# yjxiong/action-detection

Hardware: NVIDIA H100
Metric: proposals/sec (9-seg BNInception SSN fwd+bwd) (higher is better)
Workload: dtype f32 via split f16 operands (hi+lo, 3 wgmma MMAs per product) / f32 accumulate; f32 storage

## Files before the change

### action-detection_b200/csrc/engine.cu

```cuda
#include <cstdio>
#include <cstdlib>
#include <algorithm>
#include <cstring>
#include <map>
#include <string>
#include <vector>

#include <cuda_profiler_api.h>

#include "../../include/ssnb.h"
#include "common.cuh"
#include "umma_conv.cuh"

namespace ssnb {

std::atomic<long long> g_launches{0};
static thread_local std::string t_error;
void set_thread_error(const std::string& s) { t_error = s; }
const std::string& thread_error() { return t_error; }

thread_local bool t_timing = false;
thread_local LaunchTag t_tag;
struct TimingMark { const char* what; LaunchTag tag; std::string op; cudaEvent_t ev; };
static thread_local std::vector<TimingMark> t_marks;
static thread_local std::vector<cudaEvent_t> t_event_pool;
static thread_local std::string t_report;
static cudaEvent_t timing_event() {
  if (!t_event_pool.empty()) { cudaEvent_t e = t_event_pool.back(); t_event_pool.pop_back(); return e; }
  cudaEvent_t e = nullptr;
  cudaEventCreate(&e);
  return e;
}
void timing_mark(const char* what, cudaStream_t s) {
  TimingMark m{what, t_tag, t_tag.op ? t_tag.op : "", timing_event()};
  m.tag.op = nullptr;
  if (m.ev && cudaEventRecord(m.ev, s) == cudaSuccess) t_marks.push_back(m);
  else cudaGetLastError();
  t_tag.flop = 0.0; t_tag.op = nullptr; t_tag.tiles = 0; t_tag.block_n = 0;
}

static bool timing_close() {
  t_timing = false;
  if (t_marks.empty()) return false;
  if (cudaEventSynchronize(t_marks.back().ev) != cudaSuccess) { cudaGetLastError(); return false; }
  return true;
}

struct BlockSpec { const char* name; int c1, c3r, c3, cdr, cd1, cd2; int pool_max; int cproj; int stride; };
static const BlockSpec kBlocks[10] = {
    {"3a", 64, 64, 64, 64, 96, 96, 0, 32, 1},      {"3b", 64, 64, 96, 64, 96, 96, 0, 64, 1},
    {"3c", 0, 128, 160, 64, 96, 96, 1, 0, 2},      {"4a", 224, 64, 96, 96, 128, 128, 0, 128, 1},
    {"4b", 192, 96, 128, 96, 128, 128, 0, 128, 1}, {"4c", 160, 128, 160, 128, 160, 160, 0, 128, 1},
    {"4d", 96, 128, 192, 160, 192, 192, 0, 128, 1}, {"4e", 0, 128, 192, 192, 256, 256, 1, 0, 2},
    {"5a", 352, 192, 320, 160, 224, 224, 0, 128, 1}, {"5b", 352, 192, 320, 192, 224, 224, 1, 128, 1}};

struct ConvSpec { std::string id; int cin, cout, k, stride, pad; };

static std::vector<ConvSpec> conv_table(int in_ch) {
  std::vector<ConvSpec> v;
  v.push_back({"conv1_7x7_s2", in_ch, 64, 7, 2, 3});
  v.push_back({"conv2_3x3_reduce", 64, 64, 1, 1, 0});
  v.push_back({"conv2_3x3", 64, 192, 3, 1, 1});
  int cx = 192;
  for (const BlockSpec& b : kBlocks) {
    std::string p = std::string("inception_") + b.name + "_";
    if (b.c1) v.push_back({p + "1x1", cx, b.c1, 1, 1, 0});
    v.push_back({p + "3x3_reduce", cx, b.c3r, 1, 1, 0});
    v.push_back({p + "3x3", b.c3r, b.c3, 3, b.stride, 1});
    v.push_back({p + "double_3x3_reduce", cx, b.cdr, 1, 1, 0});
    v.push_back({p + "double_3x3_1", b.cdr, b.cd1, 3, 1, 1});
    v.push_back({p + "double_3x3_2", b.cd1, b.cd2, 3, b.stride, 1});
    if (b.cproj) v.push_back({p + "pool_proj", cx, b.cproj, 1, 1, 0});
    cx = b.c1 + b.c3 + b.cd2 + (b.cproj ? b.cproj : cx);
  }
  return v;
}

struct Buffer { std::string name; int H, W, C; size_t off = 0, goff = 0; size_t hoff = 0, ghoff = 0, plane = 0; };
struct Value { std::string name; int buf, coff, C; };
enum OpKind { OP_CONV = 0, OP_MAXPOOL = 1, OP_AVGPOOL = 2, OP_GPOOL = 3, OP_BN1 = 4 };
struct Op {
  OpKind kind; std::string id; int in_val, out_val;
  int conv = -1, k = 0, stride = 1, pad = 0;
  size_t argmax_off = 0;
  int grad_accumulate = 0;
  int wsplits = 1, wrows = 0;
  int tsplits = 1;
  size_t partial_off = 0, bias_partial_off = 0;
  UmmaConvPlan umma;
  UmmaConvPlan umma_dgrad;
  UmmaWgradPlan umma_wgrad;
  int pool_consumer = -1;
  bool folded_into_conv = false;
  bool dgrad_masks = false;
  bool bias_in_wgrad = false;
  bool dy_premasked = false;
  bool raw = false;
  int fuse_role = 0;
  int fuse_block = -1;
};
struct PackedConv { size_t wf, wd, bias, scale; size_t wf16 = 0, wd16 = 0, wplane = 0, wmax = 0; };
struct FusedBlock {
  int op1 = -1, op_r3 = -1, op_rd = -1;
  int c1 = 0, c3r = 0, cdr = 0, cx = 0;
  size_t w_fwd = 0, bias = 0, w_dg = 0;
  size_t w_fwd_plane = 0, w_dg_plane = 0, wmax = 0;
  UmmaConvPlan fwd, dgrad;
  bool enabled = false;
};

}

using namespace ssnb;

struct ssnb_engine {
  ssnb_config cfg;
  int F = 0;
  size_t esz = 4;
  size_t up_plane = 0, s2d_plane = 0, s2d_w_plane = 0;
  int* tc_flag = nullptr;
  size_t tc_flag_off = 0, wmax_off = 0;
  bool bn1_train = false;
  const float *bn1_gamma = nullptr, *bn1_beta = nullptr; float *bn1_rmean = nullptr, *bn1_rvar = nullptr, *bn1_dgamma = nullptr, *bn1_dbeta = nullptr;
  float bn1_momentum = 0.1f, bn1_eps = 1e-5f;
  size_t bn_stat_off = 0, bn_partial_off = 0;
  std::vector<ConvSpec> convs;
  std::vector<Buffer> bufs;
  std::vector<Value> vals;
  std::map<std::string, int> val_by_name;
  std::vector<Op> ops;
  std::vector<PackedConv> packed;
  std::vector<FusedBlock> fused;
  size_t ws_bytes = 0, partial_off = 0, partial_bytes = 0, bpartial_off = 0;
  size_t s2d_off = 0, s2d_w_off = 0, up_off = 0;
  bool fold_pools = true;
  bool s2d_ready = false;
  int Cs = 0;
  char* ws = nullptr;
  bool weights_ready = false;
  std::vector<float*> dw, db;
  std::vector<int> pending_finalize;
  int grad_accumulate = 0;
  std::string error;
  long long launches0 = 0;
  UmmaContext umma_ctx;

  int fail(int code, const std::string& msg) { error = msg; return code; }
  bool fast() const { return cfg.precision == SSNB_FAST_FP16; }
  bool exact_tc() const { return cfg.precision == SSNB_EXACT_TC; }
  bool tensor_cores() const { return cfg.precision != SSNB_EXACT_FP32; }
  int nplanes() const { return exact_tc() ? 2 : 1; }
  View view(int val, bool grad) const {
    const Value& v = vals[val];
    const Buffer& b = bufs[v.buf];
    View w;
    w.base = ws + (grad ? b.goff : b.off);
    w.H = b.H; w.W = b.W; w.C = v.C; w.pitch = b.C; w.coff = v.coff;
    return w;
  }
  View planes(int val, bool grad) const {
    const Value& v = vals[val];
    const Buffer& b = bufs[v.buf];
    View w;
    w.base = ws + (grad ? b.ghoff : b.hoff);
    w.H = b.H; w.W = b.W; w.C = v.C; w.pitch = b.C; w.coff = v.coff; w.lo_off = (long long)b.plane;
    return w;
  }
  View operand(int val, bool grad) const { return exact_tc() ? planes(val, grad) : view(val, grad); }
  const __half* w_fwd(const PackedConv& p) const { return (const __half*)(ws + (exact_tc() ? p.wd16 : p.wd)); }
  const __half* w_dgrad(const PackedConv& p) const { return (const __half*)(ws + (exact_tc() ? p.wf16 : p.wf)); }
  const UmmaTcOpts* tc_opts(UmmaTcOpts& t, size_t w_lo_off, void* out32, float alpha, size_t wmax) const {
    if (!exact_tc()) return nullptr;
    t.w_lo_off = (long long)w_lo_off; t.out32 = (float*)out32; t.alpha = alpha; t.alpha_dev = (const float*)(ws + wmax) + 1;
    return &t;
  }
};

namespace ssnb {

static size_t align_up(size_t v, size_t a) { return (v + a - 1) / a * a; }
static bool profiled_op(const char* env, const std::string& id) {
  const char* e = getenv(env);
  if (!e || !*e) return false;
  const std::string list = std::string(",") + e + ",";
  return list.find("," + id + ",") != std::string::npos;
}
static bool env_on(const char* name) {
  const char* v = getenv(name);
  return v && v[0] == '1';
}
static int device_sms() {
  int dev = 0, sms = 0;
  if (cudaGetDevice(&dev) != cudaSuccess || cudaDeviceGetAttribute(&sms, cudaDevAttrMultiProcessorCount, dev) != cudaSuccess || sms <= 0) {
    cudaGetLastError();
    return 132;
  }
  return sms;
}

static int pool_out(int h, int k, int s, int p) {
  int o = (h + 2 * p - k + s - 1) / s + 1;
  if ((o - 1) * s >= h + p) --o;
  return o;
}

static int add_buffer(ssnb_engine* e, const std::string& name, int H, int W, int C) {
  e->bufs.push_back({name, H, W, C});
  return (int)e->bufs.size() - 1;
}
static int add_value(ssnb_engine* e, const std::string& name, int buf, int coff, int C) {
  e->vals.push_back({name, buf, coff, C});
  e->val_by_name[name] = (int)e->vals.size() - 1;
  return (int)e->vals.size() - 1;
}

static void build_graph(ssnb_engine* e) {
  const int cin = e->cfg.in_channels;
  e->convs = conv_table(cin);
  int ci = 0;
  auto conv_op = [&](int in_val, int out_val) {
    const ConvSpec& c = e->convs[ci];
    Op o; o.kind = OP_CONV; o.id = c.id; o.in_val = in_val; o.out_val = out_val; o.conv = ci;
    o.k = c.k; o.stride = c.stride; o.pad = c.pad;
    e->ops.push_back(o);
    ++ci;
  };
  auto pool_op = [&](OpKind kind, const std::string& id, int in_val, int out_val, int k, int s, int p) {
    Op o; o.kind = kind; o.id = id; o.in_val = in_val; o.out_val = out_val; o.k = k; o.stride = s; o.pad = p;
    e->ops.push_back(o);
  };
  auto whole = [&](const std::string& name, int H, int W, int C) {
    return add_value(e, name, add_buffer(e, name, H, W, C), 0, C);
  };
  int x = whole("data", 224, 224, cin);
  int v;
  if (e->bn1_train) {
    const int raw = whole("conv1_7x7_s2_raw", 112, 112, 64); conv_op(x, raw); e->ops.back().raw = true;
    v = whole("conv1_7x7_s2_bn", 112, 112, 64);
    pool_op(OP_BN1, "conv1_7x7_s2_bn", raw, v, 0, 1, 0); x = v;
  } else {
    v = whole("conv1_7x7_s2_bn", 112, 112, 64); conv_op(x, v); x = v;
  }
  v = whole("pool1_3x3_s2", 56, 56, 64); pool_op(OP_MAXPOOL, "pool1_3x3_s2", x, v, 3, 2, 0); x = v;
  v = whole("conv2_3x3_reduce_bn", 56, 56, 64); conv_op(x, v); x = v;
  v = whole("conv2_3x3_bn", 56, 56, 192); conv_op(x, v); x = v;
  v = whole("pool2_3x3_s2", 28, 28, 192); pool_op(OP_MAXPOOL, "pool2_3x3_s2", x, v, 3, 2, 0); x = v;
  int H = 28, cx = 192;
  for (const BlockSpec& b : kBlocks) {
    const std::string p = std::string("inception_") + b.name + "_";
    const int OHW = (b.stride == 2) ? pool_out(H, 3, 2, 0) : H;
    const int ctot = b.c1 + b.c3 + b.cd2 + (b.cproj ? b.cproj : cx);
    const int cat = add_buffer(e, p + "output", OHW, OHW, ctot);
    const int red = add_buffer(e, p + "reduce", H, H, b.c3r + b.cdr);
    int off = 0;
    if (b.c1) { v = add_value(e, p + "1x1_bn", cat, off, b.c1); conv_op(x, v); off += b.c1; }
    int r3 = add_value(e, p + "3x3_reduce_bn", red, 0, b.c3r); conv_op(x, r3);
    v = add_value(e, p + "3x3_bn", cat, off, b.c3); conv_op(r3, v); off += b.c3;
    int rd = add_value(e, p + "double_3x3_reduce_bn", red, b.c3r, b.cdr); conv_op(x, rd);
    int d1 = whole(p + "double_3x3_1_bn", H, H, b.cd1); conv_op(rd, d1);
    v = add_value(e, p + "double_3x3_2_bn", cat, off, b.cd2); conv_op(d1, v); off += b.cd2;
    if (b.stride == 2) {
      v = add_value(e, p + "pool", cat, off, cx);
      pool_op(OP_MAXPOOL, p + "pool", x, v, 3, 2, 0);
    } else {
      int pl = whole(p + "pool", H, H, cx);
      pool_op(b.pool_max ? OP_MAXPOOL : OP_AVGPOOL, p + "pool", x, pl, 3, 1, 1);
      v = add_value(e, p + "pool_proj_bn", cat, off, b.cproj); conv_op(pl, v);
    }
    x = add_value(e, p + "output", cat, 0, ctot);
    H = OHW; cx = ctot;
  }
  Op g; g.kind = OP_GPOOL; g.id = "global_pool"; g.in_val = x; g.out_val = -1; g.k = 7;
  e->ops.push_back(g);
}

static void plan(ssnb_engine* e) {
  const size_t F = (size_t)e->F;
  size_t off = 0;
  for (Buffer& b : e->bufs) { b.off = off; off = align_up(off + F * b.H * b.W * b.C * e->esz, 1024); }
  if (e->cfg.training)
    for (Buffer& b : e->bufs) { b.goff = off; off = align_up(off + F * b.H * b.W * b.C * e->esz, 1024); }
  if (e->exact_tc()) {
    for (Buffer& b : e->bufs) {
      if (b.C % 8) continue;
      b.plane = align_up(F * b.H * b.W * b.C * 2, 1024);
      b.hoff = off; off += 2 * b.plane;
      if (e->cfg.training) { b.ghoff = off; off += 2 * b.plane; }
    }
  }
  e->tc_flag_off = off; off = align_up(off + 256, 1024);
  if (e->bn1_train) { e->bn_stat_off = off; off = align_up(off + 4 * 64 * 4, 1024); e->bn_partial_off = off; off = align_up(off + (size_t)1200 * 2 * 64 * 4, 1024); }
  for (Op& o : e->ops)
    if (o.kind == OP_MAXPOOL) {
      const Buffer& ob = e->bufs[e->vals[o.out_val].buf];
      o.argmax_off = off;
      off = align_up(off + F * ob.H * ob.W * e->vals[o.out_val].C, 1024);
    }
  e->packed.resize(e->convs.size());
  for (size_t i = 0; i < e->convs.size(); ++i) {
    const ConvSpec& c = e->convs[i];
    const size_t n = (size_t)c.cout * c.cin * c.k * c.k;
    e->packed[i].wf = off; off = align_up(off + n * e->esz, 1024);
    e->packed[i].wd = off; off = align_up(off + n * e->esz, 1024);
    e->packed[i].bias = off; off = align_up(off + c.cout * 4, 256);
    e->packed[i].scale = off; off = align_up(off + c.cout * 4, 256);
    if (e->exact_tc()) {
      e->packed[i].wplane = align_up(n * 2, 1024);
      e->packed[i].wf16 = off; off += 2 * e->packed[i].wplane;
      e->packed[i].wd16 = off; off += 2 * e->packed[i].wplane;
    }
  }
  if (e->exact_tc()) {
    e->wmax_off = off;
    for (size_t i = 0; i < e->convs.size(); ++i) e->packed[i].wmax = off + i * 8;
    off = align_up(off + (e->convs.size() + 16) * 8, 1024);
  }
  size_t pmax = 0;
  if (e->cfg.training) {
    std::vector<char> written(e->vals.size(), 0);
    for (int i = (int)e->ops.size() - 1; i >= 0; --i) {
      Op& o = e->ops[i];
      o.grad_accumulate = written[o.in_val];
      written[o.in_val] = 1;
      if (o.kind == OP_CONV) {
        const ConvSpec& c = e->convs[o.conv];
        const Buffer& ob = e->bufs[e->vals[o.out_val].buf];
        const long long M = (long long)F * ob.H * ob.W;
        const int taps = c.k * c.k;
        const bool flat = c.cin < 16;
        const long long tiles = (long long)((c.cout + 63) / 64) * (flat ? (taps * c.cin + 63) / 64 : ((c.cin + 63) / 64) * taps);
        long long splits = (592 + tiles - 1) / tiles;
        if (splits > 128) splits = 128;
        while (splits > 1 && M / splits < 256) --splits;
        long long rows = (M + splits - 1) / splits;
        rows = (rows + 15) / 16 * 16;
        splits = (M + rows - 1) / rows;
        o.wsplits = (int)splits; o.wrows = (int)rows;
        {
          const int chunks = (c.cin + 63) / 64, n_tiles = (chunks + 3) / 4, block_n = ((chunks + n_tiles - 1) / n_tiles) * 64;
          const int tpc = std::max(1, 4 / (block_n / 64));
          const int ctas = ((c.cout + 127) / 128) * n_tiles * ((taps + tpc - 1) / tpc);
          o.tsplits = std::max(o.wsplits, std::min(128, std::max(1, device_sms() / ctas)));
        }
        if (e->tensor_cores()) splits = std::max<long long>(splits, o.tsplits);
        const size_t need = (size_t)splits * taps * c.cout * c.cin * 4;
        if (need > pmax) pmax = need;
      }
    }
  }
  if (e->tensor_cores()) {
    for (int i = 0; i < (int)e->ops.size(); ++i) {
      const Op& o = e->ops[i];
      if (o.kind != OP_CONV || o.k != 1) continue;
      const std::string& id = o.id;
      const std::string suf = "_3x3_reduce";
      if (id.size() < suf.size() || id.compare(id.size() - suf.size(), suf.size(), suf) != 0 || id.find("double") != std::string::npos) continue;
      const std::string pre = id.substr(0, id.size() - suf.size() + 1);
      FusedBlock fb; fb.op_r3 = i;
      for (int j = 0; j < (int)e->ops.size(); ++j) {
        if (e->ops[j].id == pre + "1x1") fb.op1 = j;
        if (e->ops[j].id == pre + "double_3x3_reduce") fb.op_rd = j;
      }
      if (fb.op_rd < 0) continue;
      fb.cx = e->convs[o.conv].cin; fb.c3r = e->convs[o.conv].cout; fb.cdr = e->convs[e->ops[fb.op_rd].conv].cout;
      fb.c1 = fb.op1 >= 0 ? e->convs[e->ops[fb.op1].conv].cout : 0;
      const int n = fb.c1 + fb.c3r + fb.cdr, kf = (fb.c1 + 63) / 64 * 64 + fb.c3r + fb.cdr;
      fb.w_fwd_plane = align_up((size_t)n * fb.cx * 2, 1024); fb.w_dg_plane = align_up((size_t)fb.cx * kf * 2, 1024);
      if (e->exact_tc()) fb.w_fwd_plane = fb.w_dg_plane = std::max(fb.w_fwd_plane, fb.w_dg_plane);
      fb.w_fwd = off; off += e->nplanes() * fb.w_fwd_plane;
      fb.bias = off; off = align_up(off + (size_t)n * 4, 256);
      fb.w_dg = off; off += e->nplanes() * fb.w_dg_plane;
      if (e->exact_tc()) {
        if (e->fused.size() >= 16) continue;
        fb.wmax = e->wmax_off + (e->convs.size() + e->fused.size()) * 8;
        for (int j : {fb.op1, fb.op_r3, fb.op_rd}) if (j >= 0) e->packed[e->ops[j].conv].wmax = fb.wmax;
      }
      e->fused.push_back(fb);
    }
  }
  if (e->tensor_cores()) {
    for (int i = 0; i < (int)e->ops.size(); ++i) {
      Op& po = e->ops[i];
      if (po.kind != OP_MAXPOOL || po.k != 3 || po.stride != 2 || po.pad != 0) continue;
      int producer = -1, consumers = 0;
      for (int j = 0; j < (int)e->ops.size(); ++j) {
        if (e->ops[j].out_val == po.in_val && e->ops[j].kind == OP_CONV) producer = j;
        if (e->ops[j].in_val == po.in_val) ++consumers;
      }
      if (producer >= 0 && consumers == 1 && e->vals[po.in_val].C % (e->fast() ? 8 : 4) == 0) { e->ops[producer].pool_consumer = i; po.folded_into_conv = true; }
    }
    auto operand_region = [&](size_t bytes, size_t& plane) {
      const size_t at = off;
      if (e->exact_tc()) { plane = align_up(bytes, 1024); off += 2 * plane; }
      else off = align_up(off + bytes, 1024);
      return at;
    };
    e->Cs = (4 * e->cfg.in_channels + 7) / 8 * 8;
    e->s2d_off = operand_region(F * 112 * 112 * 4 * e->Cs * 2, e->s2d_plane);
    e->s2d_w_off = operand_region((size_t)16 * 64 * e->Cs * 2, e->s2d_w_plane);
    if (e->cfg.training) {
      size_t up = 0;
      for (const Op& o : e->ops)
        if (o.kind == OP_CONV && o.stride == 2 && o.conv != 0) {
          const Buffer& ib = e->bufs[e->vals[o.in_val].buf];
          up = std::max(up, F * ib.H * ib.W * (size_t)e->convs[o.conv].cout * 2);
        }
      e->up_off = operand_region(up, e->up_plane);
      pmax = std::max(pmax, (size_t)128 * 16 * 64 * e->Cs * 4);
    }
  }
  e->partial_off = off; e->partial_bytes = pmax; off = align_up(off + pmax, 1024);
  if (e->cfg.training)
    for (Op& o : e->ops)
      if (o.kind == OP_CONV) {
        const ConvSpec& c = e->convs[o.conv];
        const int nsplit = e->tensor_cores() ? std::max(o.wsplits, o.tsplits) : o.wsplits;
        size_t need = (size_t)nsplit * c.k * c.k * c.cout * c.cin * 4;
        if (o.conv == 0 && e->tensor_cores()) need = std::max(need, (size_t)128 * 16 * 64 * e->Cs * 4);
        o.partial_off = off; off = align_up(off + need, 1024);
        o.bias_partial_off = off; off = align_up(off + (size_t)std::max(nsplit, 128) * c.cout * 4, 256);
      }
  e->bpartial_off = off; off = align_up(off + (size_t)1024 * 512 * 4, 1024);
  e->ws_bytes = off;
}

#define DISPATCH(e, call_f, call_h) ((e)->fast() ? (call_h) : (call_f))

static double conv_flops(const ssnb_engine* e, const Op& o) {
  const ConvSpec& c = e->convs[o.conv];
  const Buffer& ob = e->bufs[e->vals[o.out_val].buf];
  return 2.0 * e->F * ob.H * ob.W * (double)c.cout * c.cin * c.k * c.k;
}
static inline void tag_next(int phase, double flop, const char* op = nullptr) { t_tag.phase = phase; t_tag.flop = flop; t_tag.op = op; }
static thread_local std::string t_fused_name;
static const char* fused_name(const ssnb_engine* e, const FusedBlock& fb) {
  if (!t_timing) return nullptr;
  t_fused_name.clear();
  for (int j : {fb.op1, fb.op_r3, fb.op_rd})
    if (j >= 0) t_fused_name += (t_fused_name.empty() ? "" : "+") + e->ops[j].id;
  return t_fused_name.c_str();
}

static int tc_split_value(ssnb_engine* e, int val, bool grad, float scale, cudaStream_t s) {
  if (!e->exact_tc() || !e->bufs[e->vals[val].buf].plane) return 0;
  return launch_split_view(e->view(val, grad), e->F, scale, e->planes(val, grad), grad ? e->tc_flag : nullptr, s);
}

static int run_fwd_impl(ssnb_engine* e, const Op& o, const float* input_nchw, float* feat, cudaStream_t s);
static int run_fwd(ssnb_engine* e, const Op& o, const float* input_nchw, float* feat, cudaStream_t s) {
  tag_next(0, 0.0);
  if (o.kind == OP_CONV && o.umma.enabled) {
    if (o.conv == 0 && !e->s2d_ready) {
      const View in = e->view(o.in_val, false);
      __half* s2d = (__half*)(e->ws + e->s2d_off);
      if (int rc = e->exact_tc() ? launch_nhwc_to_s2d_split(in, e->F, s2d, (long long)e->s2d_plane, e->Cs, s) : launch_nhwc_to_s2d(in, e->F, s2d, e->Cs, s))
        return rc;
    }
    tag_next(0, conv_flops(e, o), o.id.c_str());
    return umma_conv_launch(e->umma_ctx, o.umma, s);
  }
  if (o.kind == OP_BN1) {
    if (!e->bn1_gamma || !e->bn1_beta) { set_thread_error("bn1_train engine: call ssnb_set_bn1 first"); return SSNB_ESTATE; }
    return launch_bn_train_fwd(e->view(o.in_val, false), e->view(o.out_val, false), e->exact_tc() ? e->planes(o.out_val, false) : View(), e->F, e->bn1_gamma,
                               e->bn1_beta, e->bn1_eps, e->bn1_momentum, e->bn1_rmean, e->bn1_rvar, (float*)(e->ws + e->bn_stat_off),
                               (float*)(e->ws + e->bn_partial_off), 1200, s);
  }
  if (e->exact_tc() && (o.kind == OP_MAXPOOL || o.kind == OP_AVGPOOL) && e->bufs[e->vals[o.out_val].buf].plane) {
    const View in = e->view(o.in_val, false), out = e->view(o.out_val, false), pl = e->planes(o.out_val, false);
    if (o.kind == OP_MAXPOOL) return launch_maxpool_fwd_f4(in, out, pl, e->F, o.k, o.stride, o.pad, (uint8_t*)(e->ws + o.argmax_off), s);
    return launch_avgpool3_f4(in, out, pl, e->F, 0, s);
  }
  if (int rc = run_fwd_impl(e, o, input_nchw, feat, s)) return rc;
  return o.out_val >= 0 ? tc_split_value(e, o.out_val, false, 1.0f, s) : 0;
}

static int run_fwd_impl(ssnb_engine* e, const Op& o, const float* input_nchw, float* feat, cudaStream_t s) {
  const int F = e->F;
  if (o.kind == OP_CONV) {
    const ConvSpec& c = e->convs[o.conv];
    const View in = e->view(o.in_val, false), out = e->view(o.out_val, false);
    ConvArgs a;
    a.src = in.base; a.SH = in.H; a.SW = in.W; a.Csrc = in.C; a.src_pitch = in.pitch; a.src_coff = in.coff;
    a.dst = out.base; a.DH = out.H; a.DW = out.W; a.Cdst = out.C; a.dst_pitch = out.pitch; a.dst_coff = out.coff;
    a.wgt = e->ws + e->packed[o.conv].wf; a.bias = (const float*)(e->ws + e->packed[o.conv].bias);
    a.F = F; a.k = c.k; a.stride = c.stride; a.pad = c.pad; a.relu = o.raw ? 0 : 1; a.accumulate = 0; a.dgrad = 0;
    tag_next(0, conv_flops(e, o), o.id.c_str());
    return DISPATCH(e, launch_conv<float>(a, s), launch_conv<__half>(a, s));
  }
  if (o.kind == OP_MAXPOOL) {
    const View in = e->view(o.in_val, false), out = e->view(o.out_val, false);
    uint8_t* am = (uint8_t*)(e->ws + o.argmax_off);
    if (e->fast() && in.C % 8 == 0) return launch_maxpool_fwd_h8(in, out, F, o.k, o.stride, o.pad, am, s);
    return DISPATCH(e, launch_maxpool_fwd<float>(in, out, F, o.k, o.stride, o.pad, am, s),
                    launch_maxpool_fwd<__half>(in, out, F, o.k, o.stride, o.pad, am, s));
  }
  if (o.kind == OP_AVGPOOL) {
    const View in = e->view(o.in_val, false), out = e->view(o.out_val, false);
    if (e->fast() && in.C % 8 == 0) return launch_avgpool3_h8(in, out, F, 0, s);
    return DISPATCH(e, launch_avgpool3_fwd<float>(in, out, F, 0, s), launch_avgpool3_fwd<__half>(in, out, F, 0, s));
  }
  if (o.kind == OP_GPOOL) {
    if (!feat) return e->fail(SSNB_EINVAL, "global_pool needs the feat output pointer");
    const View in = e->view(o.in_val, false);
    return DISPATCH(e, launch_gpool_fwd<float>(in, F, feat, s), launch_gpool_fwd<__half>(in, F, feat, s));
  }
  return SSNB_EINVAL;
}

static int simt_wgrad(ssnb_engine* e, const Op& o, cudaStream_t s) {
  const ConvSpec& c = e->convs[o.conv];
  const View x = e->view(o.in_val, false), dz = e->view(o.out_val, true);
  float* partial = (float*)(e->ws + o.partial_off);
  WgradArgs w;
  w.dz = dz.base; w.OH = dz.H; w.OW = dz.W; w.Cout = dz.C; w.dz_pitch = dz.pitch; w.dz_coff = dz.coff;
  w.x = x.base; w.IH = x.H; w.IW = x.W; w.Cin = x.C; w.x_pitch = x.pitch; w.x_coff = x.coff;
  w.partial = partial; w.F = e->F; w.k = c.k; w.stride = c.stride; w.pad = c.pad;
  w.rows_per_split = o.wrows; w.splits = o.wsplits;
  tag_next(2, conv_flops(e, o), o.id.c_str());
  if (int rc = DISPATCH(e, launch_wgrad<float>(w, s), launch_wgrad<__half>(w, s))) return rc;
  const float out_scale = e->fast() ? 1.0f / e->cfg.grad_scale : 1.0f;
  return launch_wgrad_finalize(partial, o.wsplits, c.k * c.k, c.cout, c.cin, (const float*)(e->ws + e->packed[o.conv].scale), out_scale,
                               e->dw[o.conv], e->grad_accumulate, s);
}
static int simt_dgrad(ssnb_engine* e, const Op& o, cudaStream_t s) {
  const ConvSpec& c = e->convs[o.conv];
  const View dz = e->view(o.out_val, true), dx = e->view(o.in_val, true);
  ConvArgs a;
  a.src = dz.base; a.SH = dz.H; a.SW = dz.W; a.Csrc = dz.C; a.src_pitch = dz.pitch; a.src_coff = dz.coff;
  a.dst = dx.base; a.DH = dx.H; a.DW = dx.W; a.Cdst = dx.C; a.dst_pitch = dx.pitch; a.dst_coff = dx.coff;
  a.wgt = e->ws + e->packed[o.conv].wd; a.bias = nullptr;
  a.F = e->F; a.k = c.k; a.stride = c.stride; a.pad = c.pad; a.relu = 0; a.accumulate = o.grad_accumulate; a.dgrad = 1;
  tag_next(1, conv_flops(e, o), o.id.c_str());
  return DISPATCH(e, launch_conv<float>(a, s), launch_conv<__half>(a, s));
}

static int run_bwd(ssnb_engine* e, const Op& o, const float* dfeat, cudaStream_t s, bool skip_dgrad = false, bool full = false) {
  const int F = e->F;
  const float gs = e->fast() ? e->cfg.grad_scale : 1.0f;
  int rc = 0;
  tag_next(3, 0.0);
  if (o.kind == OP_GPOOL) {
    if (!dfeat) return e->fail(SSNB_EINVAL, "global_pool backward needs dfeat");
    const View din = e->view(o.in_val, true);
    const void* ym = (full && e->fold_pools && o.dgrad_masks) ? e->view(o.in_val, false).base : nullptr;
    return DISPATCH(e, launch_gpool_bwd<float>(dfeat, gs, din, F, ym, s), launch_gpool_bwd<__half>(dfeat, gs, din, F, ym, s));
  }
  if (o.kind == OP_BN1) {
    return launch_bn_train_bwd(e->view(o.in_val, false), e->view(o.out_val, true), e->view(o.out_val, false), e->view(o.in_val, true),
                               e->exact_tc() ? e->planes(o.in_val, true) : View(), e->cfg.grad_scale, e->tc_flag, F, e->bn1_gamma, (float*)(e->ws + e->bn_stat_off),
                               (float*)(e->ws + e->bn_partial_off), 1200, e->bn1_dgamma, e->bn1_dbeta, e->grad_accumulate, s);
  }
  if (o.kind == OP_MAXPOOL) {
    if (full && e->tensor_cores() && e->fold_pools && o.folded_into_conv) return 0;
    const View din = e->view(o.in_val, true), dout = e->view(o.out_val, true);
    const uint8_t* am = (const uint8_t*)(e->ws + o.argmax_off);
    if (e->exact_tc() && din.C % 4 == 0) return launch_maxpool_bwd_f4(din, dout, F, o.k, o.stride, o.pad, am, o.grad_accumulate, s);
    if (e->fast() && din.C % 8 == 0) return launch_maxpool_bwd_h8(din, dout, F, o.k, o.stride, o.pad, am, o.grad_accumulate, s);
    return DISPATCH(e, launch_maxpool_bwd<float>(din, dout, F, o.k, o.stride, o.pad, am, o.grad_accumulate, s),
                    launch_maxpool_bwd<__half>(din, dout, F, o.k, o.stride, o.pad, am, o.grad_accumulate, s));
  }
  if (o.kind == OP_AVGPOOL) {
    const View din = e->view(o.in_val, true), dout = e->view(o.out_val, true);
    if (e->exact_tc() && din.C % 4 == 0) return launch_avgpool3_f4(dout, din, View(), F, o.grad_accumulate, s);
    if (e->fast() && din.C % 8 == 0) return launch_avgpool3_h8(dout, din, F, o.grad_accumulate, s);
    return DISPATCH(e, launch_avgpool3_fwd<float>(dout, din, F, o.grad_accumulate, s),
                    launch_avgpool3_fwd<__half>(dout, din, F, o.grad_accumulate, s));
  }
  const ConvSpec& c = e->convs[o.conv];
  const View x = e->view(o.in_val, false), y = e->view(o.out_val, false), dy = e->view(o.out_val, true);
  const float* scale = (const float*)(e->ws + e->packed[o.conv].scale);
  float* bpartial = (float*)(e->ws + e->bpartial_off);
  float* dbp = (e->db.size() && e->db[o.conv]) ? e->db[o.conv] : nullptr;
  const bool want_w = e->dw.size() && e->dw[o.conv];
  const bool want_x = e->vals[o.in_val].name != "data" && !skip_dgrad;
  if (!e->tensor_cores()) {
    if (!o.raw && (rc = launch_relu_mask<float>(dy, y, F, s))) return rc;
    if (dbp) {
      const long long M = (long long)F * y.H * y.W;
      int bs = (int)((M + 4095) / 4096); if (bs > 64) bs = 64; if (bs < 1) bs = 1;
      if ((rc = launch_bias_grad<float>(dy.base, (int)M, y.C, dy.pitch, dy.coff, scale, 1.0f, bpartial, bs, dbp, e->grad_accumulate, s))) return rc;
    }
    if (want_w && (rc = simt_wgrad(e, o, s))) return rc;
    return want_x ? simt_dgrad(e, o, s) : 0;
  }

  const float gst = e->cfg.grad_scale;
  const bool tc_w = want_w && o.umma_wgrad.enabled, tc_x = want_x && o.umma_dgrad.enabled;
  const bool pre = full && e->fold_pools && o.dy_premasked;
  const bool bias_w = pre && o.bias_in_wgrad && dbp && tc_w;
  const Op* pool = (full && e->fold_pools && o.pool_consumer >= 0) ? &e->ops[o.pool_consumer] : nullptr;
  const int max_ctas = (1024 * 512 - 64) / y.C;
  if (e->fast()) {
    if (pool) rc = launch_pool_mask_bias_h8(dy, y, e->view(pool->out_val, true), F, pool->k, pool->stride, pool->pad, (const uint8_t*)(e->ws + pool->argmax_off),
                                            scale, 1.0f / gst, bpartial, max_ctas, dbp, e->grad_accumulate, s);
    else if (!bias_w) rc = launch_mask_bias_h8(dy, pre ? View() : y, F, scale, 1.0f / gst, bpartial, max_ctas, dbp, e->grad_accumulate, s);
  } else {
    const bool need_f32 = (want_w && !tc_w) || (want_x && !tc_x);
    const View pl = (tc_w || tc_x) ? e->planes(o.out_val, true) : View();
    if (o.raw) {
      if (dbp) rc = launch_mask_bias_split_f4(dy, View(), View(), gst, 0, nullptr, F, scale, 1.0f, bpartial, max_ctas, dbp, e->grad_accumulate, s);
    } else if (pre) {
      if (!bias_w && dbp) rc = launch_mask_bias_split_f4(dy, y, View(), gst, 0, nullptr, F, scale, 1.0f, bpartial, max_ctas, dbp, e->grad_accumulate, s);
    } else if (pool) {
      rc = launch_pool_mask_bias_split_f4(dy, y, e->view(pool->out_val, true), pl, gst, need_f32 ? 1 : 0, e->tc_flag, F, (const uint8_t*)(e->ws + pool->argmax_off),
                                          scale, 1.0f, bpartial, max_ctas, dbp, e->grad_accumulate, s);
    } else {
      rc = launch_mask_bias_split_f4(dy, y, pl, gst, (need_f32 || !full) ? 1 : 0, e->tc_flag, F, scale, 1.0f, bpartial, max_ctas, dbp, e->grad_accumulate, s);
    }
  }
  if (rc) return rc;
  if (tc_x && c.stride == 2 && o.conv != 0) {
    View dz = e->operand(o.out_val, true);
    for (int p = 0; p < e->nplanes(); ++p, dz.base = (char*)dz.base + dz.lo_off)
      if ((rc = launch_upsample2_zero(dz, (__half*)(e->ws + e->up_off + p * e->up_plane), x.H, x.W, F, s))) return rc;
  }
  if (tc_w) {
    float* partial = (float*)(e->ws + o.partial_off);
    float* bp = bias_w ? (float*)(e->ws + o.bias_partial_off) : nullptr;
    tag_next(2, conv_flops(e, o), o.id.c_str());
    if ((rc = umma_wgrad_launch(e->umma_ctx, o.umma_wgrad, s, bp))) return rc;
    if (full && o.conv != 0) e->pending_finalize.push_back((int)(&o - e->ops.data()));
    else if (o.conv == 0) rc = launch_wgrad_finalize_s2d(partial, o.umma_wgrad.p.splits, c.cout, c.cin, e->Cs, scale, 1.0f / gst, e->dw[o.conv], e->grad_accumulate, s);
    else rc = launch_wgrad_finalize(partial, o.umma_wgrad.p.splits, c.k * c.k, c.cout, c.cin, scale, 1.0f / gst, e->dw[o.conv], e->grad_accumulate, s,
                                    nullptr, nullptr, e->tc_flag);
    if (rc) return rc;
  } else if (want_w && (rc = simt_wgrad(e, o, s))) return rc;
  if (tc_x) {
    tag_next(1, conv_flops(e, o), o.id.c_str());
    return umma_conv_launch(e->umma_ctx, o.umma_dgrad, s, full && e->fold_pools && o.dgrad_masks);
  }
  return want_x ? simt_dgrad(e, o, s) : 0;
}

int engine_tail_view(ssnb_handle h, View* v, int* F, int* fp16) {
  if (!h->ws || !h->weights_ready) return h->fail(SSNB_ESTATE, "workspace/weights not set");
  *v = h->view(h->ops.back().in_val, false);
  *F = h->F; *fp16 = h->fast() ? 1 : 0;
  return 0;
}

}

extern "C" {

const char* ssnb_version(void) { return "libssn_b200 0.3 (sm_90a)"; }

const char* ssnb_last_error(ssnb_handle h) { return h ? h->error.c_str() : ssnb::thread_error().c_str(); }

int ssnb_num_convs(void) { return 69; }

int ssnb_conv_info(int idx, int in_channels, char* name, int name_cap, int* cin, int* cout, int* k, int* stride, int* pad) {
  std::vector<ConvSpec> t = conv_table(in_channels);
  if (idx < 0 || idx >= (int)t.size()) { set_thread_error("ssnb_conv_info: index out of range"); return SSNB_EINVAL; }
  if (name && name_cap > 0) { snprintf(name, name_cap, "%s", t[idx].id.c_str()); }
  if (cin) *cin = t[idx].cin; if (cout) *cout = t[idx].cout; if (k) *k = t[idx].k;
  if (stride) *stride = t[idx].stride; if (pad) *pad = t[idx].pad;
  return SSNB_OK;
}

int ssnb_create(const ssnb_config* cfg, ssnb_handle* out) {
  if (!cfg || !out) { set_thread_error("ssnb_create: null argument"); return SSNB_EINVAL; }
  if (cfg->frames <= 0 || cfg->in_channels <= 0 || cfg->in_channels > 64) { set_thread_error("ssnb_create: bad frames/in_channels"); return SSNB_EINVAL; }
  if (cfg->precision != SSNB_EXACT_FP32 && cfg->precision != SSNB_FAST_FP16 && cfg->precision != SSNB_EXACT_TC) { set_thread_error("ssnb_create: unknown precision"); return SSNB_EINVAL; }
  ssnb_engine* e = new ssnb_engine();
  e->cfg = *cfg;
  if (!(e->cfg.grad_scale > 0.f)) e->cfg.grad_scale = 1.0f;
  e->F = cfg->frames;
  e->bn1_train = cfg->bn1_train != 0;
  if (e->bn1_train && e->fast()) { delete e; set_thread_error("ssnb_create: bn1_train (bn_mode='partial') needs EXACT_FP32 or EXACT_TC"); return SSNB_ENOSUPPORT; }
  e->esz = e->fast() ? 2 : 4;
  build_graph(e);
  if ((int)e->convs.size() != 69) { delete e; set_thread_error("internal: conv table size"); return SSNB_ESTATE; }
  umma_context_init(e->umma_ctx);
  plan(e);
  e->launches0 = g_launches.load();
  *out = e;
  return SSNB_OK;
}

int ssnb_destroy(ssnb_handle h) {
  if (!h) return SSNB_OK;
  umma_context_destroy(h->umma_ctx);
  delete h;
  return SSNB_OK;
}

size_t ssnb_workspace_bytes(ssnb_handle h) { return h ? h->ws_bytes : 0; }

int ssnb_set_workspace(ssnb_handle h, void* dev_ptr, size_t bytes) {
  if (!h) return SSNB_EINVAL;
  if (!dev_ptr || bytes < h->ws_bytes) return h->fail(SSNB_EINVAL, "workspace too small");
  if (((uintptr_t)dev_ptr) % 1024) return h->fail(SSNB_EINVAL, "workspace must be 1024-byte aligned");
  h->ws = (char*)dev_ptr;
  h->weights_ready = false;
  if (h->tensor_cores() && cudaMemset(h->ws + h->bpartial_off, 0, 256) != cudaSuccess) { cudaGetLastError();  }
  h->tc_flag = (int*)(h->ws + h->tc_flag_off);
  if (cudaMemset(h->tc_flag, 0, 256) != cudaSuccess) cudaGetLastError();
  const bool training = h->cfg.training != 0;
  const bool use_tc = h->tensor_cores() && !env_on("SSNB_DISABLE_UMMA");
  const bool use_wgrad = use_tc && training && !env_on("SSNB_DISABLE_UMMA_WGRAD");
  const bool fuse = !env_on("SSNB_DISABLE_FUSION");
  const float gs = h->cfg.grad_scale;
  for (Op& o : h->ops) {
    o.umma.enabled = o.umma_dgrad.enabled = o.umma_wgrad.enabled = false;
    o.fuse_role = 0; o.fuse_block = -1; o.dgrad_masks = o.dy_premasked = o.bias_in_wgrad = false;
  }
  for (FusedBlock& fb : h->fused) fb.enabled = false;
  h->fold_pools = fuse && (h->fast() || (use_tc && training));
  auto tc_gate = [&](UmmaConvPlan& p) {
    if (h->exact_tc() && !p.p.tc_ok) p.enabled = false;
    return p.enabled;
  };
  for (Op& o : h->ops) {
    if (o.kind != OP_CONV || !use_tc) continue;
    const ConvSpec& c = h->convs[o.conv];
    const PackedConv& pk = h->packed[o.conv];
    UmmaTcOpts tf, tg;
    int rc = 0;
    if (o.conv == 0) {
      const int Ck = 4 * h->Cs;
      View xs; xs.base = h->ws + h->s2d_off; xs.H = 112; xs.W = 112; xs.C = Ck; xs.pitch = Ck; xs.coff = 0; xs.lo_off = (long long)h->s2d_plane;
      int dy[4], dx[4];
      for (int t = 0; t < 4; ++t) { dy[t] = t - 2; dx[t] = 0; }
      rc = umma_conv_bind_taps(h->umma_ctx, o.umma, xs, h->operand(o.out_val, false), h->F, Ck, c.cout, 4, dy, dx, (const __half*)(h->ws + h->s2d_w_off),
                               (const float*)(h->ws + pk.bias), o.raw ? 0 : 1, h->tc_opts(tf, h->s2d_w_plane, h->view(o.out_val, false).base, 1.0f, pk.wmax));
      if (rc) return h->fail(rc, "conv1 bind: " + ssnb::thread_error());
      tc_gate(o.umma);
      if (use_wgrad && (rc = umma_wgrad_bind_taps(h->umma_ctx, o.umma_wgrad, h->operand(o.out_val, true), xs, h->F, Ck, c.cout, 4, dy, dx,
                                                  (float*)(h->ws + o.partial_off), 128)))
        return h->fail(rc, "conv1 wgrad bind: " + ssnb::thread_error());
      continue;
    }
    if (c.cin % 8 != 0 || c.k * c.k > UMMA_MAX_TAPS) continue;
    rc = umma_conv_bind_fwd(h->umma_ctx, o.umma, h->operand(o.in_val, false), h->operand(o.out_val, false), h->F, c.cin, c.cout, c.k, c.pad,
                            c.stride, h->w_fwd(pk), (const float*)(h->ws + pk.bias), h->tc_opts(tf, pk.wplane, h->view(o.out_val, false).base, 1.0f, pk.wmax));
    if (rc) return h->fail(rc, "bind_fwd(" + c.id + "): " + ssnb::thread_error());
    if (!training) continue;
    const View in = h->view(o.in_val, false);
    View dz = h->operand(o.out_val, true);
    if (c.stride == 2) { dz.base = h->ws + h->up_off; dz.H = in.H; dz.W = in.W; dz.C = c.cout; dz.pitch = c.cout; dz.coff = 0; dz.lo_off = (long long)h->up_plane; }
    View dx = h->view(o.in_val, true);
    const UmmaTcOpts* og = h->tc_opts(tg, pk.wplane, dx.base, 1.0f / gs, pk.wmax);
    if (og) dx.base = nullptr;
    rc = umma_conv_bind_dgrad(h->umma_ctx, o.umma_dgrad, dz, dx, h->F, c.cin, c.cout, c.k, c.pad, h->w_dgrad(pk), o.grad_accumulate, og);
    if (rc) return h->fail(rc, "bind_dgrad(" + c.id + "): " + ssnb::thread_error());
    tc_gate(o.umma_dgrad);
    if (use_wgrad && (rc = umma_wgrad_bind(h->umma_ctx, o.umma_wgrad, h->operand(o.out_val, true), h->operand(o.in_val, false), h->F, c.cin, c.cout,
                                           c.k, c.pad, (float*)(h->ws + o.partial_off), o.tsplits, c.stride)))
      return h->fail(rc, "wgrad_bind(" + c.id + "): " + ssnb::thread_error());
  }
  for (size_t bi = 0; bi < h->fused.size() && use_tc && fuse; ++bi) {
    FusedBlock& fb = h->fused[bi];
    const Op& o3 = h->ops[fb.op_r3]; const Op& od = h->ops[fb.op_rd];
    if (!o3.umma.enabled || !od.umma.enabled) continue;
    const int nr = fb.c3r + fb.cdr;
    const View x = h->operand(o3.in_val, false);
    View red = h->operand(o3.out_val, false); red.C = nr;
    UmmaTcOpts tf, tg;
    int rc;
    if (fb.op1 >= 0) {
      const int v1 = h->ops[fb.op1].out_val;
      const UmmaTcOpts* of = h->tc_opts(tf, fb.w_fwd_plane, h->view(v1, false).base, 1.0f, fb.wmax);
      tf.out32_2 = (float*)h->view(o3.out_val, false).base;
      rc = umma_conv_bind_fused_fwd(h->umma_ctx, fb.fwd, x, h->operand(v1, false), red, h->F, fb.cx, fb.c1, nr, (const __half*)(h->ws + fb.w_fwd),
                                    (const float*)(h->ws + fb.bias), of);
    } else {
      rc = umma_conv_bind_fwd(h->umma_ctx, fb.fwd, x, red, h->F, fb.cx, nr, 1, 0, 1, (const __half*)(h->ws + fb.w_fwd), (const float*)(h->ws + fb.bias),
                              h->tc_opts(tf, fb.w_fwd_plane, h->view(o3.out_val, false).base, 1.0f, fb.wmax));
    }
    if (rc) return h->fail(rc, "fused fwd bind(" + o3.id + "): " + ssnb::thread_error());
    if (!tc_gate(fb.fwd)) continue;
    if (training) {
      View dred = h->operand(o3.out_val, true); dred.C = nr;
      const View d1 = fb.op1 >= 0 ? h->operand(h->ops[fb.op1].out_val, true) : dred;
      View dx = h->view(o3.in_val, true);
      const UmmaTcOpts* og = h->tc_opts(tg, fb.w_dg_plane, dx.base, 1.0f / gs, fb.wmax);
      if (og) dx.base = nullptr;
      rc = umma_conv_bind_fused_dgrad(h->umma_ctx, fb.dgrad, d1, dred, dx, h->F, fb.cx, fb.c1, nr, (const __half*)(h->ws + fb.w_dg), od.grad_accumulate, og);
      if (rc) return h->fail(rc, "fused dgrad bind(" + o3.id + "): " + ssnb::thread_error());
      if (!tc_gate(fb.dgrad)) continue;
      if (h->exact_tc() && cudaMemset(h->ws + fb.w_dg, 0, 2 * fb.w_dg_plane) != cudaSuccess) cudaGetLastError();
    }
    fb.enabled = true;
    const int leader = fb.op1 >= 0 ? fb.op1 : fb.op_r3;
    for (int j : {fb.op1, fb.op_r3, fb.op_rd})
      if (j >= 0) { h->ops[j].fuse_block = (int)bi; h->ops[j].fuse_role = (j == leader) ? 1 : 2; }
  }
  if (use_tc && training && fuse) {
    std::vector<int> first_consumer(h->vals.size(), -1);
    for (int i = 0; i < (int)h->ops.size(); ++i)
      if (first_consumer[h->ops[i].in_val] < 0) first_consumer[h->ops[i].in_val] = i;
    for (size_t v = 0; v < h->vals.size(); ++v) {
      const int fc = first_consumer[v];
      if (fc < 0 || h->vals[v].name == "data") continue;
      if (h->exact_tc() && !h->bufs[h->vals[v].buf].plane) continue;
      bool conv_made = false;
      for (const Op& q : h->ops) conv_made = conv_made || (q.kind == OP_CONV && h->vals[q.out_val].buf == h->vals[v].buf);
      if (!conv_made) continue;
      Op& c = h->ops[fc];
      UmmaConvPlan* dg = nullptr;
      if (c.kind == OP_CONV && c.fuse_role == 1 && h->fused[c.fuse_block].enabled) dg = &h->fused[c.fuse_block].dgrad;
      else if (c.kind == OP_CONV && c.fuse_role == 0 && c.umma_dgrad.enabled) dg = &c.umma_dgrad;
      if (dg) {
        c.dgrad_masks = true;
        if (h->exact_tc()) umma_conv_set_mask_tc(*dg, h->view((int)v, false), h->planes((int)v, true), gs, h->tc_flag);
        else umma_conv_set_mask(*dg, h->view((int)v, false));
      } else if (c.kind == OP_GPOOL && h->fast()) {
        c.dgrad_masks = true;
      }
    }
    for (Op& o : h->ops) {
      if (o.kind != OP_CONV) continue;
      int w = o.out_val;
      if (first_consumer[w] < 0) {
        const Value& ov = h->vals[o.out_val];
        for (size_t v = 0; v < h->vals.size(); ++v)
          if (h->vals[v].buf == ov.buf && h->vals[v].coff == 0 && h->vals[v].C == h->bufs[ov.buf].C && first_consumer[v] >= 0) { w = (int)v; break; }
      }
      if (first_consumer[w] >= 0 && h->ops[first_consumer[w]].dgrad_masks) o.dy_premasked = true;
      o.bias_in_wgrad = o.dy_premasked && o.conv != 0 && o.umma_wgrad.enabled;
    }
  }
  return SSNB_OK;
}

int ssnb_pack_weights(ssnb_handle h, const float* const* w, const float* const* b, const float* const* gamma,
                      const float* const* beta, const float* const* mean, const float* const* var, void* stream) {
  if (!h || !h->ws) return h ? h->fail(SSNB_ESTATE, "set_workspace first") : SSNB_EINVAL;
  cudaStream_t s = (cudaStream_t)stream;
  if (h->exact_tc() && cudaMemsetAsync(h->ws + h->wmax_off, 0, (h->convs.size() + 16) * 8, s) != cudaSuccess) return h->fail(SSNB_ECUDA, "pack_weights: memset");
  {
    struct Member { int block = -1, row = 0, col = 0; };
    std::vector<Member> member(h->convs.size());
    for (size_t bi = 0; bi < h->fused.size(); ++bi) {
      const FusedBlock& fb = h->fused[bi];
      if (!fb.enabled) continue;
      const int k1p = (fb.c1 + 63) / 64 * 64;
      int row = 0, col = 0;
      for (int j : {fb.op1, fb.op_r3, fb.op_rd}) {
        if (j < 0) continue;
        const int ci = h->ops[j].conv;
        member[ci].block = (int)bi; member[ci].row = row; member[ci].col = col;
        row += h->convs[ci].cout;
        col += (j == fb.op1) ? k1p : h->convs[ci].cout;
      }
    }
    std::vector<PackTable> pt(1);
    std::vector<SplitTable> stt(1);
    std::vector<int> pblocks(1, 0), sblocks(1, 0);
    pt[0].n = 0; pt[0].pad_ = 0; stt[0].n = 0; stt[0].pad_ = 0;
    for (size_t i = 0; i < h->convs.size(); ++i) {
      const ConvSpec& c = h->convs[i];
      const PackedConv& p = h->packed[i];
      const long long n = (long long)c.cout * c.cin * c.k * c.k;
      if (pt.back().n == PACK_MAX) { pt.emplace_back(); pt.back().n = 0; pt.back().pad_ = 0; pblocks.push_back(0); stt.emplace_back(); stt.back().n = 0; stt.back().pad_ = 0; sblocks.push_back(0); }
      const Member& mb = member[i];
      const FusedBlock* fb = mb.block >= 0 ? &h->fused[mb.block] : nullptr;
      PackEntry& q = pt.back().e[pt.back().n++];
      q.w = w[i]; q.b = b[i]; q.gamma = gamma[i]; q.beta = beta[i]; q.mean = mean[i]; q.var = var[i];
      q.wf = h->ws + p.wf; q.wd = h->ws + p.wd; q.bias = (float*)(h->ws + p.bias); q.scale = (float*)(h->ws + p.scale);
      q.absmax = h->exact_tc() ? (float*)(h->ws + p.wmax) : nullptr;
      q.cout = c.cout; q.cin = c.cin; q.k = c.k; q.block0 = pblocks.back();
      q.nofold = (h->bn1_train && i == 0) ? 1 : 0; q.pad_[0] = q.pad_[1] = q.pad_[2] = 0;
      q.bias_b = (h->exact_tc() && fb) ? (float*)(h->ws + fb->bias) + mb.row : nullptr;
      pblocks.back() += pack_ctas(c.cout, c.cin, c.k);
      if (h->exact_tc()) {
        SplitEntry& e = stt.back().e[stt.back().n++];
        e.wf = (const float*)(h->ws + p.wf); e.wd = (const float*)(h->ws + p.wd);
        e.wf16 = (__half*)(h->ws + p.wf16); e.wd16 = (__half*)(h->ws + p.wd16); e.plane_bytes = (long long)p.wplane; e.n = n;
        e.absmax = (const float*)(h->ws + p.wmax); e.inv_scale = (float*)(h->ws + p.wmax) + 1; e.block0 = sblocks.back(); e.pad_ = 0;
        e.wd16_b = nullptr; e.wf16_b = nullptr; e.b_plane_bytes = 0; e.b_pitch = 0; e.cout = c.cout;
        if (fb) {
          const int kf = (fb->c1 + 63) / 64 * 64 + fb->c3r + fb->cdr;
          e.wd16_b = (__half*)(h->ws + fb->w_fwd) + (size_t)mb.row * fb->cx;
          e.wf16_b = (__half*)(h->ws + fb->w_dg) + mb.col;
          e.b_pitch = kf;
          e.b_plane_bytes = (long long)std::max(fb->w_fwd_plane, fb->w_dg_plane);
        }
        sblocks.back() += (int)((n + 255) / 256);
      }
    }
    for (size_t k = 0; k < pt.size(); ++k) {
      int rc = h->fast() ? launch_pack_all<__half>(pt[k], pblocks[k], s) : launch_pack_all<float>(pt[k], pblocks[k], s);
      if (rc) return h->fail(rc, "pack_weights: " + ssnb::thread_error());
    }
    if (h->exact_tc())
      for (size_t k = 0; k < stt.size(); ++k)
        if (int rc = launch_split_all(stt[k], sblocks[k], s)) return h->fail(rc, "pack_weights split: " + ssnb::thread_error());
  }
  if (h->ops.size() && h->ops[0].umma.enabled) {
    const PackedConv& p = h->packed[0];
    for (int pl = 0; pl < h->nplanes(); ++pl) {
      int rc = launch_pack_conv1_s2d((const __half*)((const char*)h->w_fwd(p) + pl * p.wplane), h->convs[0].cout, h->convs[0].cin, h->Cs,
                                     (__half*)(h->ws + h->s2d_w_off + pl * h->s2d_w_plane), s);
      if (rc) return h->fail(rc, "pack conv1 s2d: " + ssnb::thread_error());
    }
  }
  for (FusedBlock& fb : h->fused) {
    if (!fb.enabled || !h->fast()) continue;
    const int k1p = (fb.c1 + 63) / 64 * 64, kf = k1p + fb.c3r + fb.cdr;
    __half* wfwd = (__half*)(h->ws + fb.w_fwd); float* bias = (float*)(h->ws + fb.bias); __half* wdg = (__half*)(h->ws + fb.w_dg);
    if (cudaMemsetAsync(wdg, 0, (size_t)fb.cx * kf * 2, s) != cudaSuccess) return h->fail(SSNB_ECUDA, "fused pack: memset");
    int row = 0, col = 0;
    for (int j : {fb.op1, fb.op_r3, fb.op_rd}) {
      if (j < 0) { continue; }
      const int ci = h->ops[j].conv, co = h->convs[ci].cout;
      cudaError_t e1 = cudaMemcpyAsync(wfwd + (size_t)row * fb.cx, h->ws + h->packed[ci].wd, (size_t)co * fb.cx * 2, cudaMemcpyDeviceToDevice, s);
      cudaError_t e2 = cudaMemcpyAsync(bias + row, h->ws + h->packed[ci].bias, (size_t)co * 4, cudaMemcpyDeviceToDevice, s);
      cudaError_t e3 = cudaMemcpy2DAsync(wdg + col, (size_t)kf * 2, h->ws + h->packed[ci].wf, (size_t)co * 2, (size_t)co * 2, fb.cx,
                                         cudaMemcpyDeviceToDevice, s);
      if (e1 != cudaSuccess || e2 != cudaSuccess || e3 != cudaSuccess) return h->fail(SSNB_ECUDA, "fused pack: copy failed");
      row += co;
      col += (j == fb.op1) ? k1p : co;
    }
  }
  h->weights_ready = true;
  return SSNB_OK;
}

int ssnb_set_bn1(ssnb_handle h, const float* gamma, const float* beta, float* running_mean, float* running_var, float* dgamma, float* dbeta,
                 float momentum, float eps) {
  if (!h) return SSNB_EINVAL;
  if (!h->bn1_train) return h->fail(SSNB_ESTATE, "engine created without bn1_train");
  if (!gamma || !beta) return h->fail(SSNB_EINVAL, "set_bn1: gamma / beta are required");
  h->bn1_gamma = gamma; h->bn1_beta = beta; h->bn1_rmean = running_mean; h->bn1_rvar = running_var; h->bn1_dgamma = dgamma; h->bn1_dbeta = dbeta;
  h->bn1_momentum = momentum; h->bn1_eps = eps;
  return SSNB_OK;
}

int ssnb_backbone_fwd(ssnb_handle h, const float* input_nchw, float* feat, void* stream) {
  if (!h || !input_nchw || !feat) return h ? h->fail(SSNB_EINVAL, "null argument") : SSNB_EINVAL;
  if (!h->ws || !h->weights_ready) return h->fail(SSNB_ESTATE, "workspace/weights not set");
  cudaStream_t s = (cudaStream_t)stream;
  const View d = h->view(h->val_by_name["data"], false);
  int rc;
  h->s2d_ready = h->tensor_cores() && h->ops[0].umma.enabled;
  if (h->s2d_ready && h->exact_tc()) rc = launch_nchw_to_s2d_split(input_nchw, h->F, d.C, d.H, d.W, (__half*)(h->ws + h->s2d_off), (long long)h->s2d_plane, h->Cs, s);
  else if (h->s2d_ready) rc = launch_nchw_to_s2d(input_nchw, h->F, d.C, d.H, d.W, (__half*)(h->ws + h->s2d_off), h->Cs, s);
  else rc = h->fast() ? launch_nchw_to_nhwc<__half>(input_nchw, h->F, d.C, d.H, d.W, d, 1.0f, s)
                    : launch_nchw_to_nhwc<float>(input_nchw, h->F, d.C, d.H, d.W, d, 1.0f, s);
  if (rc) { h->s2d_ready = false; return h->fail(rc, "input layout: " + ssnb::thread_error()); }
  for (size_t i = 0; i < h->ops.size(); ++i) {
    const Op& o = h->ops[i];
    if (o.fuse_role == 2) continue;
    const bool prof = profiled_op("SSNB_PROFILE_FWD_OPS", o.id);
    if (prof) cudaProfilerStart();
    int r;
    if (o.fuse_role == 1) {
      const FusedBlock& fb = h->fused[o.fuse_block];
      double fl = 0.0;
      for (int j : {fb.op1, fb.op_r3, fb.op_rd}) if (j >= 0) fl += conv_flops(h, h->ops[j]);
      tag_next(0, fl, fused_name(h, fb));
      r = umma_conv_launch(h->umma_ctx, fb.fwd, s);
    } else r = run_fwd(h, o, input_nchw, feat, s);
    if (prof) cudaProfilerStop();
    if (r) { h->s2d_ready = false; return h->fail(r, "fwd " + o.id + ": " + ssnb::thread_error()); }
  }
  h->s2d_ready = false;
  return SSNB_OK;
}

int ssnb_bind_grads(ssnb_handle h, float* const* dw, float* const* db) {
  if (!h) return SSNB_EINVAL;
  h->dw.assign(h->convs.size(), nullptr); h->db.assign(h->convs.size(), nullptr);
  for (size_t i = 0; i < h->convs.size(); ++i) { if (dw) h->dw[i] = dw[i]; if (db) h->db[i] = db[i]; }
  return SSNB_OK;
}

int ssnb_backbone_bwd(ssnb_handle h, const float* dfeat, float* const* dw, float* const* db, void* stream) {
  return ssnb_backbone_bwd_range(h, dfeat, dw, db, -1, 0, stream);
}

int ssnb_backbone_bwd_range(ssnb_handle h, const float* dfeat, float* const* dw, float* const* db, int op_hi, int op_lo, void* stream) {
  if (!h || (!dfeat && (op_hi < 0 || op_hi >= (int)h->ops.size() - 1))) return h ? h->fail(SSNB_EINVAL, "null argument") : SSNB_EINVAL;
  if (!h->cfg.training) return h->fail(SSNB_ESTATE, "engine created without training=1");
  if (!h->ws || !h->weights_ready) return h->fail(SSNB_ESTATE, "workspace/weights not set");
  ssnb_bind_grads(h, dw, db);
  h->pending_finalize.clear();
  cudaStream_t s = (cudaStream_t)stream;
  auto run_range = [&](int hi, int lo) -> int {
    for (int i = hi; i >= lo; --i) {
      const Op& o = h->ops[i];
      const bool prof = profiled_op("SSNB_PROFILE_BWD_OPS", o.id);
      if (prof) cudaProfilerStart();
      int rc = run_bwd(h, o, dfeat, s, o.fuse_role != 0, true);
      if (!rc && o.fuse_role == 1) {
        const FusedBlock& fb = h->fused[o.fuse_block];
        double fl = 0.0;
        for (int j : {fb.op1, fb.op_r3, fb.op_rd}) if (j >= 0) fl += conv_flops(h, h->ops[j]);
        tag_next(1, fl, fused_name(h, fb));
        rc = umma_conv_launch(h->umma_ctx, fb.dgrad, s, h->fold_pools && o.dgrad_masks);
      }
      if (prof) cudaProfilerStop();
      if (rc) return h->fail(rc, "bwd " + o.id + ": " + ssnb::thread_error());
    }
    return 0;
  };
  auto finalize = [&]() -> int {
    const float gs = h->tensor_cores() ? h->cfg.grad_scale : 1.0f;
    FinalizeTable t; t.n = 0; t.total_blocks = 0; t.flag = h->tc_flag;
    auto flush = [&]() -> int { int rc = launch_wgrad_finalize_all(t, 1.0f / gs, h->grad_accumulate, s); t.n = 0; t.total_blocks = 0; return rc; };
    for (int oi : h->pending_finalize) {
      const Op& o = h->ops[oi];
      const ConvSpec& c = h->convs[o.conv];
      FinalizeEntry& q = t.e[t.n];
      q.partial = (const float*)(h->ws + o.partial_off); q.mult = (const float*)(h->ws + h->packed[o.conv].scale); q.dw = h->dw[o.conv];
      const bool bias_w = o.dy_premasked && o.bias_in_wgrad && h->db.size() && h->db[o.conv];
      q.bias_partial = bias_w ? (const float*)(h->ws + o.bias_partial_off) : nullptr; q.db = bias_w ? h->db[o.conv] : nullptr;
      q.splits = o.umma_wgrad.p.splits; q.taps = c.k * c.k; q.Cout = c.cout; q.Cin = c.cin; q.block0 = t.total_blocks; q.pad_ = 0;
      t.total_blocks += (int)(((long long)q.taps * q.Cout * q.Cin + 255) / 256);
      if (++t.n == FIN_MAX) if (int rc = flush()) { h->pending_finalize.clear(); return h->fail(rc, "finalize: " + ssnb::thread_error()); }
    }
    h->pending_finalize.clear();
    if (int rc = flush()) return h->fail(rc, "finalize: " + ssnb::thread_error());
    return 0;
  };
  const int last = (int)h->ops.size() - 1;
  if (op_hi < 0 || op_hi > last) op_hi = last;
  if (op_lo < 0 || op_lo > op_hi) return h->fail(SSNB_EINVAL, "backbone_bwd_range: bad op range");
  if (int rc = run_range(op_hi, op_lo)) return rc;
  return finalize();
}

int ssnb_set_grad_accumulate(ssnb_handle h, int accumulate) {
  if (!h) return SSNB_EINVAL;
  h->grad_accumulate = accumulate ? 1 : 0;
  return SSNB_OK;
}

int ssnb_num_ops(ssnb_handle h) { return h ? (int)h->ops.size() : 0; }

int ssnb_op_info(ssnb_handle h, int op, char* kind, int kind_cap, char* in_name, int in_cap, char* out_name, int out_cap) {
  if (!h || op < 0 || op >= (int)h->ops.size()) return SSNB_EINVAL;
  static const char* kn[] = {"conv", "maxpool", "avgpool", "gpool", "bn"};
  const Op& o = h->ops[op];
  if (kind) snprintf(kind, kind_cap, "%s", kn[o.kind]);
  if (in_name) snprintf(in_name, in_cap, "%s", h->vals[o.in_val].name.c_str());
  if (out_name) snprintf(out_name, out_cap, "%s", o.out_val >= 0 ? h->vals[o.out_val].name.c_str() : "feat");
  return SSNB_OK;
}

int ssnb_value_shape(ssnb_handle h, const char* name, int* c, int* hh, int* ww) {
  if (!h || !name) return SSNB_EINVAL;
  auto it = h->val_by_name.find(name);
  if (it == h->val_by_name.end()) return h->fail(SSNB_EINVAL, std::string("unknown value ") + name);
  const View v = h->view(it->second, false);
  if (c) *c = v.C; if (hh) *hh = v.H; if (ww) *ww = v.W;
  return SSNB_OK;
}

int ssnb_value_write(ssnb_handle h, const char* name, int grad, const float* src_nchw, void* stream) {
  if (!h || !name || !src_nchw || !h->ws) return SSNB_EINVAL;
  auto it = h->val_by_name.find(name);
  if (it == h->val_by_name.end()) return h->fail(SSNB_EINVAL, std::string("unknown value ") + name);
  if (grad && !h->cfg.training) return h->fail(SSNB_ESTATE, "no gradient buffers");
  const View v = h->view(it->second, grad != 0);
  const float sc = (grad && h->fast()) ? h->cfg.grad_scale : 1.0f;
  int rc = h->fast() ? launch_nchw_to_nhwc<__half>(src_nchw, h->F, v.C, v.H, v.W, v, sc, (cudaStream_t)stream)
                   : launch_nchw_to_nhwc<float>(src_nchw, h->F, v.C, v.H, v.W, v, sc, (cudaStream_t)stream);
  if (!rc && h->exact_tc() && !grad) rc = tc_split_value(h, it->second, false, 1.0f, (cudaStream_t)stream);
  return rc ? h->fail(rc, ssnb::thread_error()) : SSNB_OK;
}

int ssnb_value_read(ssnb_handle h, const char* name, int grad, float* dst_nchw, void* stream) {
  if (!h || !name || !dst_nchw || !h->ws) return SSNB_EINVAL;
  auto it = h->val_by_name.find(name);
  if (it == h->val_by_name.end()) return h->fail(SSNB_EINVAL, std::string("unknown value ") + name);
  if ((grad & 1) && !h->cfg.training) return h->fail(SSNB_ESTATE, "no gradient buffers");
  if (grad & 2) {
    if (!h->exact_tc() || !h->bufs[h->vals[it->second].buf].plane) return h->fail(SSNB_ESTATE, "value has no operand planes");
    int rc = launch_planes_to_nchw(h->planes(it->second, (grad & 1) != 0), h->F, (grad & 1) ? 1.0f / h->cfg.grad_scale : 1.0f, dst_nchw, (cudaStream_t)stream);
    return rc ? h->fail(rc, ssnb::thread_error()) : SSNB_OK;
  }
  const View v = h->view(it->second, grad != 0);
  const float sc = (grad && h->fast()) ? 1.0f / h->cfg.grad_scale : 1.0f;
  int rc = h->fast() ? launch_nhwc_to_nchw<__half>(v, h->F, sc, dst_nchw, (cudaStream_t)stream)
                   : launch_nhwc_to_nchw<float>(v, h->F, sc, dst_nchw, (cudaStream_t)stream);
  return rc ? h->fail(rc, ssnb::thread_error()) : SSNB_OK;
}

int ssnb_run_op(ssnb_handle h, int op, int backward, void* stream) {
  if (!h || op < 0 || op >= (int)h->ops.size()) return SSNB_EINVAL;
  if (!h->ws || !h->weights_ready) return h->fail(SSNB_ESTATE, "workspace/weights not set");
  const Op& o = h->ops[op];
  if (o.kind == OP_GPOOL) return h->fail(SSNB_ENOSUPPORT, "run_op: global_pool runs through backbone_fwd/bwd");
  int rc = backward ? run_bwd(h, o, nullptr, (cudaStream_t)stream) : run_fwd(h, o, nullptr, nullptr, (cudaStream_t)stream);
  return rc ? h->fail(rc, o.id + ": " + ssnb::thread_error()) : SSNB_OK;
}

int ssnb_grad_overflow(ssnb_handle h, int clear) {
  if (!h) return -1;
  if (!h->tc_flag) return 0;
  int v = 0;
  if (cudaMemcpy(&v, h->tc_flag, sizeof(int), cudaMemcpyDeviceToHost) != cudaSuccess) { cudaGetLastError(); return -1; }
  if (v && clear) cudaMemset(h->tc_flag, 0, sizeof(int));
  return v ? 1 : 0;
}

int ssnb_timing_begin(void* stream) {
  for (TimingMark& m : ssnb::t_marks) ssnb::t_event_pool.push_back(m.ev);
  ssnb::t_marks.clear();
  ssnb::t_tag = LaunchTag();
  ssnb::t_timing = true;
  ssnb::timing_mark("(begin)", (cudaStream_t)stream);
  return SSNB_OK;
}

const char* ssnb_timing_report(void) {
  ssnb::t_report.clear();
  if (!ssnb::timing_close()) return ssnb::t_report.c_str();
  struct Agg { int n = 0; double ms = 0, flop = 0; };
  std::map<std::pair<std::string, int>, Agg> agg;
  for (size_t i = 1; i < ssnb::t_marks.size(); ++i) {
    float ms = 0.f;
    if (cudaEventElapsedTime(&ms, ssnb::t_marks[i - 1].ev, ssnb::t_marks[i].ev) != cudaSuccess) { cudaGetLastError(); continue; }
    Agg& a = agg[{ssnb::t_marks[i].what, ssnb::t_marks[i].tag.phase}];
    a.n += 1; a.ms += ms; a.flop += ssnb::t_marks[i].tag.flop;
  }
  char line[256];
  for (const auto& kv : agg) {
    snprintf(line, sizeof line, "%s\t%d\t%d\t%.6f\t%.0f\n", kv.first.first.c_str(), kv.first.second, kv.second.n, kv.second.ms, kv.second.flop);
    ssnb::t_report += line;
  }
  return ssnb::t_report.c_str();
}

const char* ssnb_timing_launches(void) {
  ssnb::t_report.clear();
  if (!ssnb::timing_close()) return ssnb::t_report.c_str();
  char line[512];
  for (size_t i = 1; i < ssnb::t_marks.size(); ++i) {
    const ssnb::TimingMark& m = ssnb::t_marks[i];
    float ms = 0.f;
    if (cudaEventElapsedTime(&ms, ssnb::t_marks[i - 1].ev, m.ev) != cudaSuccess) { cudaGetLastError(); continue; }
    snprintf(line, sizeof line, "%s\t%d\t%s\t%.6f\t%.0f\t%d\t%d\n", m.what, m.tag.phase, m.op.empty() ? "-" : m.op.c_str(), ms, m.tag.flop,
             m.tag.tiles, m.tag.block_n);
    ssnb::t_report += line;
  }
  return ssnb::t_report.c_str();
}

int64_t ssnb_launch_count(ssnb_handle h) { return h ? (int64_t)(g_launches.load() - h->launches0) : 0; }
int64_t ssnb_global_launch_count(void) { return (int64_t)g_launches.load(); }

}
```

### action-detection_b200/csrc/umma_conv.cu

```cuda
#include <cstdio>
#include <cstdlib>
#include <cstring>
#include <algorithm>

#include "umma_conv.cuh"
#include "umma_dev.cuh"
#include "umma_epi32.cuh"

namespace ssnb {

namespace {

using namespace umma;
constexpr int MAX_STAGES = 8;
constexpr int PIPE_BYTES = 192 * 1024;
constexpr int A_BYTES = BLOCK_M * BLOCK_K * 2;
constexpr int NUM_THREADS = 384;
constexpr int N_STEP = 16;
constexpr int MAX_BLOCK_N = 128;
constexpr int EPI_COLS = 16;
constexpr int EPI_PITCH = EPI_COLS + 4;
constexpr int EPI_BYTES = BLOCK_M * EPI_PITCH * 4;
constexpr int BAR_BYTES = 256;
constexpr int SMEM_BYTES = PIPE_BYTES + 2 * EPI_BYTES + BAR_BYTES + 1024 ;
constexpr int ORDER_BAR = 1;
constexpr int EPI_BAR = 3;
static_assert(SMEM_BYTES <= 227 * 1024, "shared memory per block");

struct TileCoord { int w0, h0, f0, n0; };
__device__ __forceinline__ TileCoord decode_tile(const UmmaConvParams& p, int tile) {
  TileCoord t;
  const int nt = tile % p.n_tiles;
  int m = tile / p.n_tiles;
  t.n0 = nt * p.block_n;
  t.w0 = (m % p.tiles_w) * p.bw; m /= p.tiles_w;
  t.h0 = (m % p.tiles_h) * p.bh; m /= p.tiles_h;
  t.f0 = m * p.bf;
  return t;
}

__device__ __forceinline__ void epilogue_chunk(const UmmaConvParams& p, const uint32_t* r, int col, uint4* dst, const uint4& o0,
                                               const uint4& o1, const uint4& y0, const uint4& y1) {
  float v[16];
#pragma unroll
  for (int j = 0; j < 16; ++j) v[j] = __uint_as_float(r[j]);
  if (p.bias) {
#pragma unroll
    for (int j = 0; j < 16; ++j) v[j] += __ldg(p.bias + col + j);
  }
  if (p.accumulate) {
    const __half2* h0 = reinterpret_cast<const __half2*>(&o0);
    const __half2* h1 = reinterpret_cast<const __half2*>(&o1);
#pragma unroll
    for (int j = 0; j < 4; ++j) {
      float2 a = __half22float2(h0[j]), b = __half22float2(h1[j]);
      v[2 * j] += a.x; v[2 * j + 1] += a.y; v[8 + 2 * j] += b.x; v[8 + 2 * j + 1] += b.y;
    }
  }
  if (p.relu) {
#pragma unroll
    for (int j = 0; j < 16; ++j) v[j] = fmaxf(v[j], 0.f);
  }
  if (p.mask_y) {
    const __half2* a0 = reinterpret_cast<const __half2*>(&y0);
    const __half2* a1 = reinterpret_cast<const __half2*>(&y1);
#pragma unroll
    for (int j = 0; j < 4; ++j) {
      const float2 ya = __half22float2(a0[j]), yb = __half22float2(a1[j]);
      if (!(ya.x > 0.f)) v[2 * j] = 0.f;
      if (!(ya.y > 0.f)) v[2 * j + 1] = 0.f;
      if (!(yb.x > 0.f)) v[8 + 2 * j] = 0.f;
      if (!(yb.y > 0.f)) v[8 + 2 * j + 1] = 0.f;
    }
  }
  uint4 q0, q1;
  __half2* g0 = reinterpret_cast<__half2*>(&q0);
  __half2* g1 = reinterpret_cast<__half2*>(&q1);
#pragma unroll
  for (int j = 0; j < 4; ++j) { g0[j] = __floats2half2_rn(v[2 * j], v[2 * j + 1]); g1[j] = __floats2half2_rn(v[8 + 2 * j], v[8 + 2 * j + 1]); }
  dst[0] = q0; dst[1] = q1;
}

__device__ __forceinline__ void epilogue_row_chunk(const UmmaConvParams& p, const TileCoord& t, int row, int col, const float* st) {
  const int rw = row % p.bw, rh = (row / p.bw) % p.bh, rf = row / (p.bw * p.bh);
  const int w = t.w0 + rw, h = t.h0 + rh, f = t.f0 + rf;
  const int os = p.out_stride;
  const bool valid = (rf < p.bf) && (w < p.W) && (h < p.H) && (f < p.F) && (w % os == 0) && (h % os == 0);
  if (!valid || col >= p.Cout) return;
  const long long opix = (long long)(f * p.OH + h / os) * p.OW + w / os;
  uint32_t r[16];
#pragma unroll
  for (int j = 0; j < 4; ++j) {
    const float4 q = reinterpret_cast<const float4*>(st)[j];
    r[4 * j] = __float_as_uint(q.x); r[4 * j + 1] = __float_as_uint(q.y); r[4 * j + 2] = __float_as_uint(q.z); r[4 * j + 3] = __float_as_uint(q.w);
  }
  const bool d1 = col < p.n_split;
  if (p.out_f32) {
    const float alpha = p.alpha * (p.alpha_dev ? __ldg(p.alpha_dev) : 1.0f);
    float* o32 = d1 ? p.out32 + opix * p.out_pitch + p.out_coff + col : p.out32_2 + opix * p.out2_pitch + p.out2_coff - p.n_split + col;
    __half* hi = d1 ? p.out_hi : p.out_hi2;
    if (hi) hi += d1 ? opix * p.out_pitch + p.out_coff + col : opix * p.out2_pitch + p.out2_coff - p.n_split + col;
    const float* m32 = p.mask32 ? p.mask32 + opix * p.mask32_pitch + p.mask32_coff + col : nullptr;
    store_chunk32(p, alpha, r, p.bias + col, o32, hi, m32, d1 ? p.out_lo_off : p.out_lo_off2);
    return;
  }
  uint4* dst = reinterpret_cast<uint4*>(d1 ? p.out + opix * p.out_pitch + p.out_coff + col : p.out2 + opix * p.out2_pitch + p.out2_coff - p.n_split + col);
  uint4 o0 = {}, o1 = {}, y0 = {}, y1 = {};
  if (p.accumulate) { o0 = dst[0]; o1 = dst[1]; }
  if (p.mask_y) {
    const uint4* my = reinterpret_cast<const uint4*>(p.mask_y + opix * p.mask_pitch + p.mask_coff + col);
    y0 = __ldg(my); y1 = __ldg(my + 1);
  }
  epilogue_chunk(p, r, col, dst, o0, o1, y0, y1);
}

template <int BN, int NK>
__device__ __forceinline__ void mma_k(float* d0, float* d1, uint32_t sa, uint32_t sb) {
#pragma unroll
  for (int k = 0; k < NK; ++k) {
    const uint64_t bdesc = make_desc_sw128(sb + k * MMA_K * 2);
    wgmma<BN, 0, 0>(d0, make_desc_sw128(sa + k * MMA_K * 2), bdesc);
    wgmma<BN, 0, 0>(d1, make_desc_sw128(sa + 64 * 128 + k * MMA_K * 2), bdesc);
  }
}

template <int BN, int NK>
__device__ __forceinline__ void mma_stage(float* d0, float* d1, uint32_t sa, uint32_t sb, uint32_t b_bytes, bool split) {
  if (split) {
    mma_k<BN, NK>(d0, d1, sa + A_BYTES, sb);
    mma_k<BN, NK>(d0, d1, sa, sb + b_bytes);
  }
  mma_k<BN, NK>(d0, d1, sa, sb);
}

__device__ __forceinline__ void ring_advance(uint32_t& stage, uint32_t& phase, int n, int stages) {
  const uint32_t s = stage + (uint32_t)n;
  phase ^= (s / (uint32_t)stages) & 1u;
  stage = s % (uint32_t)stages;
}

template <int BN>
__global__ void __launch_bounds__(NUM_THREADS, 1)
umma_conv_kernel(const __grid_constant__ CUtensorMap tmap_a, const __grid_constant__ CUtensorMap tmap_a2,
                 const __grid_constant__ CUtensorMap tmap_b, const __grid_constant__ CUtensorMap tmap_a_lo,
                 const __grid_constant__ CUtensorMap tmap_a2_lo, const __grid_constant__ CUtensorMap tmap_b_lo,
                 const __grid_constant__ UmmaConvParams p) {
  extern __shared__ uint8_t smem_raw[];
  uint8_t* smem = reinterpret_cast<uint8_t*>((reinterpret_cast<uintptr_t>(smem_raw) + 1023) & ~(uintptr_t)1023);
  const int STAGES = p.stages, STAGE_BYTES = p.stage_bytes;
  uint64_t* bars = reinterpret_cast<uint64_t*>(smem + PIPE_BYTES + 2 * EPI_BYTES);
  uint64_t* full_bar = bars;
  uint64_t* empty_bar = bars + MAX_STAGES;

  const int wg = __shfl_sync(0xffffffffu, (int)threadIdx.x / 128, 0);
  const int total_tiles = p.tiles_w * p.tiles_h * p.tiles_f * p.n_tiles;
  const bool split = p.nseg > 1;
  const int nplanes = split ? 2 : 1;
  const uint32_t b_bytes = (uint32_t)p.block_n * BLOCK_K * 2;
  const int ksteps = p.ntaps * p.kchunks;

  if (threadIdx.x == 0) {
    asm volatile("prefetch.tensormap [%0];" ::"l"(reinterpret_cast<uint64_t>(&tmap_a)) : "memory");
    asm volatile("prefetch.tensormap [%0];" ::"l"(reinterpret_cast<uint64_t>(&tmap_a2)) : "memory");
    asm volatile("prefetch.tensormap [%0];" ::"l"(reinterpret_cast<uint64_t>(&tmap_b)) : "memory");
    for (int i = 0; i < STAGES; ++i) { mbar_init(&full_bar[i], 1); mbar_init(&empty_bar[i], 1); }
    asm volatile("fence.mbarrier_init.release.cluster;" ::: "memory");
  }
  __syncthreads();

  if (wg == 0) {
    producer_regs();
    if (threadIdx.x == 0) {
      uint32_t stage = 0, phase = 0;
      const uint32_t a_bytes = (uint32_t)(p.bw * p.bh * p.bf) * BLOCK_K * 2;
      const uint32_t tx_bytes = (a_bytes + b_bytes) * nplanes;
      for (int tile = blockIdx.x; tile < total_tiles; tile += gridDim.x) {
        const TileCoord t = decode_tile(p, tile);
        for (int tap = 0; tap < p.ntaps; ++tap) {
          for (int kc = 0; kc < p.kchunks; ++kc) {
            mbar_wait(&empty_bar[stage], phase ^ 1);
            uint8_t* sa = smem + stage * STAGE_BYTES;
            uint8_t* sb = sa + nplanes * A_BYTES;
            mbar_expect_tx(&full_bar[stage], tx_bytes);
            for (int pl = 0; pl < nplanes; ++pl) {
              if (kc < p.kchunks_a1)
                tma_load_4d(sa + pl * A_BYTES, pl ? &tmap_a_lo : &tmap_a, &full_bar[stage], kc * BLOCK_K, t.w0 * p.a_stride + p.tap_dx[tap],
                            t.h0 * p.a_stride + p.tap_dy[tap], t.f0);
              else
                tma_load_4d(sa + pl * A_BYTES, pl ? &tmap_a2_lo : &tmap_a2, &full_bar[stage], (kc - p.kchunks_a1) * BLOCK_K, t.w0 + p.tap_dx[tap],
                            t.h0 + p.tap_dy[tap], t.f0);
              tma_load_3d(sb + pl * b_bytes, pl ? &tmap_b_lo : &tmap_b, &full_bar[stage], kc * BLOCK_K, t.n0, tap);
            }
            if (++stage == STAGES) { stage = 0; phase ^= 1; }
          }
        }
      }
    }
  } else {
    consumer_regs();
    const int cw = wg - 1, row = threadIdx.x & 127;
    const int warp = row / 32, lane = row & 31;
    float* epi = reinterpret_cast<float*>(smem + PIPE_BYTES + cw * EPI_BYTES);
    const int my_tiles = (total_tiles - (int)blockIdx.x + (int)gridDim.x - 1) / (int)gridDim.x;
    uint32_t stage = 0, phase = 0;
    if (cw) ring_advance(stage, phase, ksteps, STAGES);
    for (int j = cw; j < my_tiles; j += 2) {
      const TileCoord t = decode_tile(p, (int)blockIdx.x + j * (int)gridDim.x);
      float acc[2][BN / 2];
#pragma unroll
      for (int b = 0; b < 2; ++b)
#pragma unroll
        for (int i = 0; i < BN / 2; ++i) acc[b][i] = 0.f;
      if (j > 0) named_bar_sync(ORDER_BAR + cw, 256);
      uint32_t prev = 0;
      int kc = 0;
      for (int ks = 0; ks < ksteps; ++ks) {
        mbar_wait(&full_bar[stage], phase);
        const uint32_t sa = smem_u32(smem + stage * STAGE_BYTES);
        const uint32_t sb = sa + nplanes * A_BYTES;
        const int kvalid = kc < p.kchunks_a1 ? p.K1 - kc * BLOCK_K : p.K - p.K1 - (kc - p.kchunks_a1) * BLOCK_K;
        const int nk = kvalid >= BLOCK_K ? BLOCK_K / MMA_K : (kvalid + MMA_K - 1) / MMA_K;
        wgmma_fence();
        switch (nk) {
          case 1: mma_stage<BN, 1>(acc[0], acc[1], sa, sb, b_bytes, split); break;
          case 2: mma_stage<BN, 2>(acc[0], acc[1], sa, sb, b_bytes, split); break;
          case 3: mma_stage<BN, 3>(acc[0], acc[1], sa, sb, b_bytes, split); break;
          default: mma_stage<BN, BLOCK_K / MMA_K>(acc[0], acc[1], sa, sb, b_bytes, split); break;
        }
        wgmma_commit();
        wgmma_wait<1>();
        if (ks > 0 && row == 0) mbar_arrive(&empty_bar[prev]);
        prev = stage;
        if (++stage == STAGES) { stage = 0; phase ^= 1; }
        if (++kc == p.kchunks) kc = 0;
      }
      if (j + 1 < my_tiles) named_bar_arrive(ORDER_BAR + (cw ^ 1), 256);
      wgmma_wait<0>();
      if (row == 0) mbar_arrive(&empty_bar[prev]);
      ring_advance(stage, phase, ksteps, STAGES);
#pragma unroll
      for (int sl = 0; sl < (BN + EPI_COLS - 1) / EPI_COLS; ++sl) {
        named_bar_sync(EPI_BAR + cw, 128);
#pragma unroll
        for (int b = 0; b < 2; ++b)
#pragma unroll
          for (int i = 0; i < EPI_COLS / 2; i += 2) {
            const int ai = sl * (EPI_COLS / 2) + i;
            if (ai < BN / 2) {
              const int r = b * 64 + warp * 16 + (lane >> 2) + 8 * ((i >> 1) & 1);
              const int c = 8 * (i >> 2) + 2 * (lane & 3);
              *reinterpret_cast<float2*>(epi + r * EPI_PITCH + c) = make_float2(acc[b][ai], acc[b][ai + 1]);
            }
          }
        named_bar_sync(EPI_BAR + cw, 128);
#pragma unroll
        for (int c = 0; c < EPI_COLS; c += 16)
          if (sl * EPI_COLS + c < BN) epilogue_row_chunk(p, t, row, t.n0 + sl * EPI_COLS + c, epi + row * EPI_PITCH + c);
      }
    }
  }
}

typedef CUresult (*EncodeTiledFn)(CUtensorMap*, CUtensorMapDataType, cuuint32_t, void*, const cuuint64_t*, const cuuint64_t*,
                                  const cuuint32_t*, const cuuint32_t*, CUtensorMapInterleave, CUtensorMapSwizzle,
                                  CUtensorMapL2promotion, CUtensorMapFloatOOBfill);

int resolve_encode(UmmaContext& ctx) {
  if (ctx.encode_tiled) return 0;
  void* fn = nullptr;
  cudaDriverEntryPointQueryResult q;
  cudaError_t e = cudaGetDriverEntryPoint("cuTensorMapEncodeTiled", &fn, cudaEnableDefault, &q);
  if (e != cudaSuccess || q != cudaDriverEntryPointSuccess || !fn) {
    cudaGetLastError();
    set_thread_error("cuTensorMapEncodeTiled not available from the driver");
    return 2;
  }
  ctx.encode_tiled = fn;
  int dev = 0, sms = 132;
  if (cudaGetDevice(&dev) == cudaSuccess) cudaDeviceGetAttribute(&sms, cudaDevAttrMultiProcessorCount, dev);
  ctx.num_sms = sms;
  return 0;
}

int encode(UmmaContext& ctx, CUtensorMap* m, int rank, void* addr, const cuuint64_t* dims, const cuuint64_t* strides,
           const cuuint32_t* box, int spatial_stride = 1) {
  cuuint32_t es[5] = {1, (cuuint32_t)spatial_stride, (cuuint32_t)spatial_stride, 1, 1};
  CUresult r = reinterpret_cast<EncodeTiledFn>(ctx.encode_tiled)(m, CU_TENSOR_MAP_DATA_TYPE_FLOAT16, (cuuint32_t)rank, addr, dims, strides,
                                                                box, es, CU_TENSOR_MAP_INTERLEAVE_NONE, CU_TENSOR_MAP_SWIZZLE_128B,
                                                                CU_TENSOR_MAP_L2_PROMOTION_L2_256B, CU_TENSOR_MAP_FLOAT_OOB_FILL_NONE);
  if (r != CUDA_SUCCESS) {
    char buf[128];
    snprintf(buf, sizeof buf, "cuTensorMapEncodeTiled failed (CUresult %d, rank %d)", (int)r, rank);
    set_thread_error(buf);
    return 2;
  }
  return 0;
}

void pick_box(int W, int& bw, int& bh, int& bf) {
  if (W % 8 == 0 && W >= 56) { bw = 8; bh = 8; bf = 2; }
  else if (W % 4 == 0) { bw = 4; bh = 4; bf = 8; }
  else if (W % 2 == 0) { bw = 2; bh = 2; bf = 32; }
  else if (W <= 8) { bw = W; bh = 1; bf = BLOCK_M / W; }
  else { bw = 1; bh = 1; bf = 128; }
}

int bind_common(UmmaContext& ctx, UmmaConvPlan& plan, View a, View o, int F, int K, int N, int ntaps, int out_stride, const __half* w,
                int a_stride = 1, const UmmaTcOpts* tc = nullptr) {
  plan.enabled = false;
  if (int rc = resolve_encode(ctx)) return rc;
  if (a_stride == 2) {
    View ao = a; ao.H = o.H; ao.W = o.W;
    if (int rc = bind_common(ctx, plan, ao, o, F, K, N, ntaps, 1, w, 1, tc)) return rc;
    plan.enabled = false;
    UmmaConvParams& q = plan.p;
    q.a_stride = 2;
    cuuint64_t dims[4] = {(cuuint64_t)K, (cuuint64_t)a.W, (cuuint64_t)a.H, (cuuint64_t)F};
    cuuint64_t str[3] = {(cuuint64_t)a.pitch * 2, (cuuint64_t)a.W * a.pitch * 2, (cuuint64_t)a.H * a.W * a.pitch * 2};
    cuuint32_t box[4] = {(cuuint32_t)BLOCK_K, (cuuint32_t)(2 * q.bw), (cuuint32_t)(2 * q.bh), (cuuint32_t)q.bf};
    if (int rc = encode(ctx, &plan.tmap_a, 4, reinterpret_cast<__half*>(a.base) + a.coff, dims, str, box, 2)) return rc;
    plan.tmap_a_lo = plan.tmap_a;
    if (a.lo_off)
      if (int rc = encode(ctx, &plan.tmap_a_lo, 4, reinterpret_cast<__half*>(reinterpret_cast<char*>(a.base) + a.lo_off) + a.coff, dims, str, box, 2)) return rc;
    plan.tmap_a2 = plan.tmap_a; plan.tmap_a2_lo = plan.tmap_a_lo;
    plan.enabled = true;
    return 0;
  }
  if ((a.H + out_stride - 1) / out_stride != o.H || (a.W + out_stride - 1) / out_stride != o.W) { set_thread_error("umma conv: geometry mismatch"); return 1; }
  if (K % 8 || N % 16 || a.pitch % 8 || a.coff % 8 || o.pitch % 8 || o.coff % 8 || ntaps > UMMA_MAX_TAPS) {
    set_thread_error("umma conv: unsupported channel alignment"); return 1; }
  UmmaConvParams& p = plan.p;
  memset(&p, 0, sizeof(p));
  p.W = a.W; p.H = a.H; p.F = F;
  pick_box(a.W, p.bw, p.bh, p.bf);
  p.tiles_w = (a.W + p.bw - 1) / p.bw; p.tiles_h = (a.H + p.bh - 1) / p.bh; p.tiles_f = (F + p.bf - 1) / p.bf;
  p.n_tiles = (N + MAX_BLOCK_N - 1) / MAX_BLOCK_N;
  p.block_n = (((N + p.n_tiles - 1) / p.n_tiles) + N_STEP - 1) / N_STEP * N_STEP;
  p.kchunks = (K + BLOCK_K - 1) / BLOCK_K;
  p.K = K;
  p.ntaps = ntaps;
  p.out = reinterpret_cast<__half*>(o.base); p.out_pitch = o.pitch; p.out_coff = o.coff; p.Cout = N;
  p.out_stride = out_stride; p.OH = o.H; p.OW = o.W; p.a_stride = 1; p.mask_y = nullptr; p.mask_pitch = 0; p.mask_coff = 0;
  p.kchunks_a1 = (K + BLOCK_K - 1) / BLOCK_K; p.K1 = K; p.n_split = 1 << 30; p.out2 = p.out; p.out2_pitch = o.pitch; p.out2_coff = o.coff;
  {
    cuuint64_t dims[4] = {(cuuint64_t)K, (cuuint64_t)a.W, (cuuint64_t)a.H, (cuuint64_t)F};
    cuuint64_t str[3] = {(cuuint64_t)a.pitch * 2, (cuuint64_t)a.W * a.pitch * 2, (cuuint64_t)a.H * a.W * a.pitch * 2};
    cuuint32_t box[4] = {(cuuint32_t)BLOCK_K, (cuuint32_t)p.bw, (cuuint32_t)p.bh, (cuuint32_t)p.bf};
    if (int rc = encode(ctx, &plan.tmap_a, 4, reinterpret_cast<__half*>(a.base) + a.coff, dims, str, box)) return rc;
    plan.tmap_a_lo = plan.tmap_a;
    if (a.lo_off)
      if (int rc = encode(ctx, &plan.tmap_a_lo, 4, reinterpret_cast<__half*>(reinterpret_cast<char*>(a.base) + a.lo_off) + a.coff, dims, str, box)) return rc;
  }
  {
    cuuint64_t dims[3] = {(cuuint64_t)K, (cuuint64_t)N, (cuuint64_t)ntaps};
    cuuint64_t str[2] = {(cuuint64_t)K * 2, (cuuint64_t)N * K * 2};
    cuuint32_t box[3] = {(cuuint32_t)BLOCK_K, (cuuint32_t)p.block_n, 1};
    if (int rc = encode(ctx, &plan.tmap_b, 3, const_cast<__half*>(w), dims, str, box)) return rc;
    plan.b_lo_off = tc ? tc->w_lo_off : 0;
    plan.tmap_b_lo = plan.tmap_b;
    if (plan.b_lo_off)
      if (int rc = encode(ctx, &plan.tmap_b_lo, 3, reinterpret_cast<__half*>(reinterpret_cast<char*>(const_cast<__half*>(w)) + plan.b_lo_off), dims, str, box)) return rc;
  }
  plan.tmap_a2 = plan.tmap_a; plan.tmap_a2_lo = plan.tmap_a_lo;
  p.nseg = tc ? 3 : 1; p.out_f32 = tc ? 1 : 0;
  p.stage_bytes = ((A_BYTES + p.block_n * BLOCK_K * 2) * (tc ? 2 : 1) + 1023) / 1024 * 1024;
  p.stages = PIPE_BYTES / p.stage_bytes; if (p.stages > MAX_STAGES) p.stages = MAX_STAGES;
  p.alpha = tc ? tc->alpha : 1.0f; p.alpha_dev = tc ? tc->alpha_dev : nullptr;
  p.mask32 = nullptr; p.mask32_pitch = 0; p.mask32_coff = 0; p.plane_scale = 1.0f; p.flag = nullptr;
  p.out32 = tc ? tc->out32 : nullptr; p.out_hi = tc ? reinterpret_cast<__half*>(o.base) : nullptr; p.out_lo_off = tc ? o.lo_off : 0;
  p.out32_2 = p.out32; p.out_hi2 = p.out_hi; p.out_lo_off2 = p.out_lo_off;
  if (tc && (!tc->out32 || !a.lo_off || !tc->w_lo_off)) { set_thread_error("umma conv: split-operand bind needs operand planes and an fp32 output"); return 1; }
  plan.enabled = true;
  return 0;
}

void mark_tc_ok(UmmaConvPlan& plan, int W, bool two_sources) {
  UmmaConvParams& p = plan.p;
  p.tc_ok = 0;
  if (!plan.enabled || p.a_stride != 1 || p.out_stride != 1) return;
  if (!(p.ntaps == 1 || p.ntaps == 4 || p.ntaps == 9)) return;
  if (p.kchunks_a1 != p.kchunks && (p.ntaps != 1 || !two_sources)) return;
  if (p.out_pitch % 16 || p.out_coff % 16 || p.out2_pitch % 16 || p.out2_coff % 16 || p.n_split % 16 || (p.bias && p.n_tiles * p.block_n > 1024)) return;
  if (W < 7) return;
  p.tc_ok = 1;
}

}

int umma_resolve_encode(UmmaContext& ctx) { return resolve_encode(ctx); }
int umma_encode_f16(UmmaContext& ctx, CUtensorMap* m, int rank, void* addr, const cuuint64_t* dims,
                    const cuuint64_t* strides, const cuuint32_t* box, int spatial_stride) {
  return encode(ctx, m, rank, addr, dims, strides, box, spatial_stride);
}

void umma_context_init(UmmaContext&) {}
void umma_context_destroy(UmmaContext&) {}

int umma_conv_bind_taps(UmmaContext& ctx, UmmaConvPlan& plan, View in, View out, int F, int cin, int cout, int ntaps,
                        const int* dy, const int* dx, const __half* w_tap_n_k, const float* bias, int relu, const UmmaTcOpts* tc) {
  if (int rc = bind_common(ctx, plan, in, out, F, cin, cout, ntaps, 1, w_tap_n_k, 1, tc)) return rc;
  for (int t = 0; t < ntaps; ++t) { plan.p.tap_dy[t] = dy[t]; plan.p.tap_dx[t] = dx[t]; }
  plan.p.bias = bias; plan.p.relu = relu; plan.p.accumulate = 0;
  mark_tc_ok(plan, in.W, false);
  return 0;
}

int umma_conv_bind_fwd(UmmaContext& ctx, UmmaConvPlan& plan, View in, View out, int F, int cin, int cout, int k, int pad,
                       int stride, const __half* w_tap_n_k, const float* bias, const UmmaTcOpts* tc) {
  const char* st = getenv("SSNB_TMA_STRIDED");
  const bool strided = stride == 2 && !(st && st[0] == '0');
  if (int rc = strided ? bind_common(ctx, plan, in, out, F, cin, cout, k * k, 1, w_tap_n_k, 2, tc)
                       : bind_common(ctx, plan, in, out, F, cin, cout, k * k, stride, w_tap_n_k, 1, tc)) return rc;
  for (int r = 0; r < k; ++r)
    for (int s = 0; s < k; ++s) { plan.p.tap_dy[r * k + s] = r - pad; plan.p.tap_dx[r * k + s] = s - pad; }
  plan.p.bias = bias; plan.p.relu = 1; plan.p.accumulate = 0;
  mark_tc_ok(plan, in.W, false);
  return 0;
}

int umma_conv_bind_dgrad(UmmaContext& ctx, UmmaConvPlan& plan, View dz, View dx, int F, int cin, int cout, int k, int pad,
                         const __half* w_tap_k_n, int accumulate, const UmmaTcOpts* tc) {
  if (int rc = bind_common(ctx, plan, dz, dx, F, cout, cin, k * k, 1, w_tap_k_n, 1, tc)) return rc;
  for (int r = 0; r < k; ++r)
    for (int s = 0; s < k; ++s) { plan.p.tap_dy[r * k + s] = pad - r; plan.p.tap_dx[r * k + s] = pad - s; }
  plan.p.bias = nullptr; plan.p.relu = 0; plan.p.accumulate = accumulate;
  mark_tc_ok(plan, dz.W, false);
  return 0;
}

int umma_conv_bind_fused_fwd(UmmaContext& ctx, UmmaConvPlan& plan, View in, View out1, View out2, int F, int cin, int n1, int n2,
                             const __half* w_n_k, const float* bias, const UmmaTcOpts* tc) {
  View o = out1; o.C = n1 + n2;
  if (out1.H != out2.H || out1.W != out2.W || n1 % 16 || n2 % 16 || out2.pitch % 8 || out2.coff % 8) { set_thread_error("fused fwd: bad views"); return 1; }
  if (int rc = bind_common(ctx, plan, in, o, F, cin, n1 + n2, 1, 1, w_n_k, 1, tc)) return rc;
  plan.p.tap_dy[0] = 0; plan.p.tap_dx[0] = 0;
  plan.p.bias = bias; plan.p.relu = 1; plan.p.accumulate = 0;
  plan.p.n_split = n1; plan.p.out2 = reinterpret_cast<__half*>(out2.base); plan.p.out2_pitch = out2.pitch; plan.p.out2_coff = out2.coff;
  if (tc) {
    if (!tc->out32_2) { set_thread_error("fused fwd: the split-operand bind needs both fp32 destinations"); return 1; }
    plan.p.out32_2 = tc->out32_2; plan.p.out_hi2 = reinterpret_cast<__half*>(out2.base); plan.p.out_lo_off2 = out2.lo_off;
  }
  mark_tc_ok(plan, in.W, false);
  return 0;
}

int umma_conv_bind_fused_dgrad(UmmaContext& ctx, UmmaConvPlan& plan, View dz1, View dz2, View dx, int F, int cin, int k1, int k2,
                               const __half* w_n_k, int accumulate, const UmmaTcOpts* tc) {
  const int k1p = (k1 + BLOCK_K - 1) / BLOCK_K * BLOCK_K;
  View a = k1 ? dz1 : dz2;
  if (int rc = bind_common(ctx, plan, a, dx, F, k1 ? k1 : k2, cin, 1, 1, w_n_k, 1, tc)) return rc;
  UmmaConvParams& p = plan.p;
  p.tap_dy[0] = 0; p.tap_dx[0] = 0; p.bias = nullptr; p.relu = 0; p.accumulate = accumulate;
  if (k1) {
    if (dz2.H != dz1.H || dz2.W != dz1.W || dz2.pitch % 8 || dz2.coff % 8 || k2 % 8) { set_thread_error("fused dgrad: bad views"); return 1; }
    cuuint64_t dims[4] = {(cuuint64_t)k2, (cuuint64_t)dz2.W, (cuuint64_t)dz2.H, (cuuint64_t)F};
    cuuint64_t str[3] = {(cuuint64_t)dz2.pitch * 2, (cuuint64_t)dz2.W * dz2.pitch * 2, (cuuint64_t)dz2.H * dz2.W * dz2.pitch * 2};
    cuuint32_t box[4] = {(cuuint32_t)BLOCK_K, (cuuint32_t)p.bw, (cuuint32_t)p.bh, (cuuint32_t)p.bf};
    if (int rc = encode(ctx, &plan.tmap_a2, 4, reinterpret_cast<__half*>(dz2.base) + dz2.coff, dims, str, box)) { plan.enabled = false; return rc; }
    p.kchunks_a1 = k1p / BLOCK_K; p.K1 = k1; p.K = k1 + k2;
    p.kchunks = p.kchunks_a1 + (k2 + BLOCK_K - 1) / BLOCK_K;
    cuuint64_t bd[3] = {(cuuint64_t)(k1p + k2), (cuuint64_t)cin, 1};
    cuuint64_t bs[2] = {(cuuint64_t)(k1p + k2) * 2, (cuuint64_t)cin * (k1p + k2) * 2};
    cuuint32_t bb[3] = {(cuuint32_t)BLOCK_K, (cuuint32_t)p.block_n, 1};
    if (int rc = encode(ctx, &plan.tmap_b, 3, const_cast<__half*>(w_n_k), bd, bs, bb)) { plan.enabled = false; return rc; }
    plan.tmap_b_lo = plan.tmap_b;
    if (plan.b_lo_off)
      if (int rc = encode(ctx, &plan.tmap_b_lo, 3, reinterpret_cast<__half*>(reinterpret_cast<char*>(const_cast<__half*>(w_n_k)) + plan.b_lo_off), bd, bs, bb)) {
        plan.enabled = false; return rc; }
    if (tc && !dz2.lo_off) { set_thread_error("fused dgrad: the split-operand bind needs the second source's operand planes"); plan.enabled = false; return 1; }
    plan.tmap_a2_lo = plan.tmap_a2;
    if (dz2.lo_off)
      if (int rc = encode(ctx, &plan.tmap_a2_lo, 4, reinterpret_cast<__half*>(reinterpret_cast<char*>(dz2.base) + dz2.lo_off) + dz2.coff, dims, str, box)) {
        plan.enabled = false; return rc; }
  }
  mark_tc_ok(plan, a.W, k1 != 0);
  return 0;
}

void umma_conv_set_mask(UmmaConvPlan& plan, View y) {
  plan.mask_y = reinterpret_cast<const __half*>(y.base); plan.mask_pitch = y.pitch; plan.mask_coff = y.coff;
}

void umma_conv_set_mask_tc(UmmaConvPlan& plan, View y32, View dplanes, float plane_scale, int* flag) {
  plan.mask32 = reinterpret_cast<const float*>(y32.base); plan.mask32_pitch = y32.pitch; plan.mask32_coff = y32.coff;
  plan.mask_planes = reinterpret_cast<__half*>(dplanes.base); plan.mask_planes_lo = dplanes.lo_off;
  plan.mask_plane_scale = plane_scale; plan.mask_flag = flag;
}

namespace {
template <int BN>
int launch_bn(const UmmaConvPlan& plan, const UmmaConvParams& p, int grid, cudaStream_t s) {
  static bool attr_set[64] = {};
  auto kern = umma_conv_kernel<BN>;
  int dev = 0;
  cudaGetDevice(&dev);
  if (dev < 0 || dev >= 64 || !attr_set[dev]) {
    if (cudaFuncSetAttribute(kern, cudaFuncAttributeMaxDynamicSharedMemorySize, SMEM_BYTES) != cudaSuccess) {
      set_thread_error("umma conv: cannot raise dynamic shared memory limit"); cudaGetLastError(); return 2; }
    if (dev >= 0 && dev < 64) attr_set[dev] = true;
  }
  kern<<<grid, NUM_THREADS, SMEM_BYTES, s>>>(plan.tmap_a, plan.tmap_a2, plan.tmap_b, plan.tmap_a_lo, plan.tmap_a2_lo, plan.tmap_b_lo, p);
  SSNB_LAUNCH_CHECK("umma_conv_kernel");
  return 0;
}
}

int umma_conv_launch(UmmaContext& ctx, const UmmaConvPlan& plan, cudaStream_t s, bool mask) {
  if (!plan.enabled) { set_thread_error("umma conv: plan not bound"); return 3; }
  UmmaConvParams p = plan.p;
  if (mask && plan.mask_y) { p.mask_y = plan.mask_y; p.mask_pitch = plan.mask_pitch; p.mask_coff = plan.mask_coff; }
  if (mask && p.out_f32 && plan.mask32) {
    p.mask32 = plan.mask32; p.mask32_pitch = plan.mask32_pitch; p.mask32_coff = plan.mask32_coff;
    p.out_hi = plan.mask_planes; p.out_lo_off = plan.mask_planes_lo; p.plane_scale = plan.mask_plane_scale; p.flag = plan.mask_flag;
  }
  if (p.out_f32 && (p.mask_y || p.out_stride != 1)) { set_thread_error("umma conv: the fp32 epilogue takes its mask through mask32 and has no sampling"); return 3; }
  const int total = p.tiles_w * p.tiles_h * p.tiles_f * p.n_tiles;
  const int grid = total < ctx.num_sms ? total : ctx.num_sms;
  t_tag.tiles = total; t_tag.block_n = p.block_n;
  switch (p.block_n) {
    case 16: return launch_bn<16>(plan, p, grid, s);
    case 32: return launch_bn<32>(plan, p, grid, s);
    case 48: return launch_bn<48>(plan, p, grid, s);
    case 64: return launch_bn<64>(plan, p, grid, s);
    case 80: return launch_bn<80>(plan, p, grid, s);
    case 96: return launch_bn<96>(plan, p, grid, s);
    case 112: return launch_bn<112>(plan, p, grid, s);
    case 128: return launch_bn<128>(plan, p, grid, s);
  }
  set_thread_error("umma conv: unsupported tile width"); return 3;
}

}
```

### action-detection_b200/csrc/umma_conv.cuh

```cuda
#pragma once
#include <cuda.h>
#include <cuda_fp16.h>
#include <cuda_runtime.h>

#include "common.cuh"

namespace ssnb {

constexpr int UMMA_MAX_TAPS = 16;

struct UmmaContext {
  void* encode_tiled = nullptr;
  int num_sms = 132;
};

struct UmmaConvParams {
  int W, H, F;
  int bw, bh, bf;
  int tiles_w, tiles_h, tiles_f;
  int n_tiles, block_n;
  int stages, stage_bytes;
  int kchunks, ntaps, K;
  int tap_dy[UMMA_MAX_TAPS], tap_dx[UMMA_MAX_TAPS];
  __half* out; int out_pitch, out_coff, Cout;
  int out_stride, OH, OW;
  int a_stride;
  const float* bias;
  int relu, accumulate;
  int kchunks_a1, K1;
  int n_split;
  __half* out2; int out2_pitch, out2_coff;
  int tc_ok;
  const __half* mask_y; int mask_pitch, mask_coff;
  int nseg, out_f32;
  float alpha;
  const float* alpha_dev;
  float* out32; __half* out_hi; long long out_lo_off;
  float* out32_2; __half* out_hi2; long long out_lo_off2;
  const float* mask32; int mask32_pitch, mask32_coff;
  float plane_scale; int* flag;
};

struct UmmaConvPlan {
  bool enabled = false;
  const __half* mask_y = nullptr; int mask_pitch = 0, mask_coff = 0;
  CUtensorMap tmap_a, tmap_a2, tmap_b;
  CUtensorMap tmap_a_lo, tmap_a2_lo, tmap_b_lo;
  long long b_lo_off = 0;
  const float* mask32 = nullptr; int mask32_pitch = 0, mask32_coff = 0;
  __half* mask_planes = nullptr; long long mask_planes_lo = 0; float mask_plane_scale = 1.0f; int* mask_flag = nullptr;
  UmmaConvParams p;
};

struct UmmaTcOpts { long long w_lo_off = 0; float* out32 = nullptr; float alpha = 1.0f; const float* alpha_dev = nullptr; float* out32_2 = nullptr; };
void umma_context_init(UmmaContext& ctx);
void umma_context_destroy(UmmaContext& ctx);
int umma_conv_bind_fwd(UmmaContext& ctx, UmmaConvPlan& plan, View in, View out, int F, int cin, int cout, int k, int pad,
                       int stride, const __half* w_tap_n_k, const float* bias, const UmmaTcOpts* tc = nullptr);
int umma_conv_bind_taps(UmmaContext& ctx, UmmaConvPlan& plan, View in, View out, int F, int cin, int cout, int ntaps,
                        const int* dy, const int* dx, const __half* w_tap_n_k, const float* bias, int relu, const UmmaTcOpts* tc = nullptr);
int umma_conv_bind_dgrad(UmmaContext& ctx, UmmaConvPlan& plan, View dz, View dx, int F, int cin, int cout, int k, int pad,
                         const __half* w_tap_k_n, int accumulate, const UmmaTcOpts* tc = nullptr);
int umma_conv_bind_fused_fwd(UmmaContext& ctx, UmmaConvPlan& plan, View in, View out1, View out2, int F, int cin, int n1, int n2,
                             const __half* w_n_k, const float* bias, const UmmaTcOpts* tc = nullptr);
int umma_conv_bind_fused_dgrad(UmmaContext& ctx, UmmaConvPlan& plan, View dz1, View dz2, View dx, int F, int cin, int k1, int k2,
                               const __half* w_n_k, int accumulate, const UmmaTcOpts* tc = nullptr);
int umma_conv_launch(UmmaContext& ctx, const UmmaConvPlan& plan, cudaStream_t s, bool mask = false);
void umma_conv_set_mask(UmmaConvPlan& plan, View y);
void umma_conv_set_mask_tc(UmmaConvPlan& plan, View y32, View dplanes, float plane_scale, int* flag);

int umma_resolve_encode(UmmaContext& ctx);
int umma_encode_f16(UmmaContext& ctx, CUtensorMap* m, int rank, void* addr, const cuuint64_t* dims,
                    const cuuint64_t* strides, const cuuint32_t* box, int spatial_stride = 1);

struct UmmaWgradParams {
  int W, H, F;
  int bw, bh, bf;
  int tiles_w, tiles_h, tiles_f;
  int ptiles_per_split, splits;
  int ntaps, tap_dy[UMMA_MAX_TAPS], tap_dx[UMMA_MAX_TAPS];
  int Cout, Cin, m_tiles, n_tiles, block_n;
  int x_stride;
  float* bias_partial;
  int taps_per_cta, tap_groups;
  int stages, stage_bytes;
  float* partial;
  int nseg;
};
struct UmmaWgradPlan {
  bool enabled = false;
  CUtensorMap tmap_dz, tmap_x;
  CUtensorMap tmap_dz_lo, tmap_x_lo;
  UmmaWgradParams p;
};
int umma_wgrad_bind(UmmaContext& ctx, UmmaWgradPlan& plan, View dz, View x, int F, int cin, int cout, int k, int pad,
                    float* partial, int max_splits, int x_stride = 1);
int umma_wgrad_bind_taps(UmmaContext& ctx, UmmaWgradPlan& plan, View dz, View x, int F, int cin, int cout, int ntaps,
                         const int* dy, const int* dx, float* partial, int max_splits, int x_stride = 1);
int umma_wgrad_launch(UmmaContext& ctx, const UmmaWgradPlan& plan, cudaStream_t s, float* bias_partial = nullptr);

}
```

### action-detection_b200/csrc/umma_dev.cuh

```cuda
#pragma once
#include <cuda.h>
#include <cuda_fp16.h>
#include <cuda_runtime.h>
#include <stdint.h>

namespace ssnb {
namespace umma {

constexpr int BLOCK_M = 128;
constexpr int BLOCK_K = 64;
constexpr int MMA_K = 16;
constexpr int MMA_N = 64;

__device__ __forceinline__ uint32_t smem_u32(const void* p) { return (uint32_t)__cvta_generic_to_shared(p); }

__device__ __forceinline__ void mbar_init(uint64_t* bar, uint32_t count) {
  asm volatile("mbarrier.init.shared::cta.b64 [%0], %1;" ::"r"(smem_u32(bar)), "r"(count) : "memory");
}
__device__ __forceinline__ void mbar_expect_tx(uint64_t* bar, uint32_t bytes) {
  asm volatile("mbarrier.arrive.expect_tx.shared::cta.b64 _, [%0], %1;" ::"r"(smem_u32(bar)), "r"(bytes) : "memory");
}
__device__ __forceinline__ void mbar_arrive(uint64_t* bar) {
  asm volatile("mbarrier.arrive.shared::cta.b64 _, [%0];" ::"r"(smem_u32(bar)) : "memory");
}
__device__ __forceinline__ bool mbar_try_wait(uint64_t* bar, uint32_t parity) {
  uint32_t ok;
  asm volatile(
      "{\n\t.reg .pred p;\n\t"
      "mbarrier.try_wait.parity.shared::cta.b64 p, [%1], %2;\n\t"
      "selp.b32 %0, 1, 0, p;\n\t}"
      : "=r"(ok)
      : "r"(smem_u32(bar)), "r"(parity)
      : "memory");
  return ok != 0;
}
__device__ __forceinline__ void mbar_wait(uint64_t* bar, uint32_t parity) {
  if (mbar_try_wait(bar, parity)) return;
  const long long t0 = clock64();
  while (!mbar_try_wait(bar, parity)) {
    if (clock64() - t0 > 4000000000LL) __trap();
  }
}

__device__ __forceinline__ void tma_load_4d(void* dst, const CUtensorMap* map, uint64_t* bar, int c0, int c1, int c2, int c3) {
  asm volatile(
      "cp.async.bulk.tensor.4d.shared::cluster.global.mbarrier::complete_tx::bytes [%0], [%1, {%3, %4, %5, %6}], [%2];" ::"r"(
          smem_u32(dst)),
      "l"(reinterpret_cast<uint64_t>(map)), "r"(smem_u32(bar)), "r"(c0), "r"(c1), "r"(c2), "r"(c3)
      : "memory");
}
__device__ __forceinline__ void tma_load_3d(void* dst, const CUtensorMap* map, uint64_t* bar, int c0, int c1, int c2) {
  asm volatile(
      "cp.async.bulk.tensor.3d.shared::cluster.global.mbarrier::complete_tx::bytes [%0], [%1, {%3, %4, %5}], [%2];" ::"r"(
          smem_u32(dst)),
      "l"(reinterpret_cast<uint64_t>(map)), "r"(smem_u32(bar)), "r"(c0), "r"(c1), "r"(c2)
      : "memory");
}

__device__ __forceinline__ uint64_t make_desc_sw128(uint32_t saddr, uint32_t lbo_bytes = 16) {
  uint64_t d = 0;
  d |= (uint64_t)((saddr >> 4) & 0x3FFF);
  d |= (uint64_t)((lbo_bytes >> 4) & 0x3FFF) << 16;
  d |= (uint64_t)(1024 >> 4) << 32;
  d |= (uint64_t)1 << 62;
  return d;
}

__device__ __forceinline__ void wgmma_fence() { asm volatile("wgmma.fence.sync.aligned;" ::: "memory"); }
__device__ __forceinline__ void wgmma_commit() { asm volatile("wgmma.commit_group.sync.aligned;" ::: "memory"); }
template <int N>
__device__ __forceinline__ void wgmma_wait() { asm volatile("wgmma.wait_group.sync.aligned %0;" ::"n"(N) : "memory"); }

template <int TA, int TB>
__device__ __forceinline__ void wgmma_n16(float* d, uint64_t adesc, uint64_t bdesc) {
  asm volatile(
      "{\n\t.reg .pred p;\n\tsetp.ne.b32 p, 1, 0;\n\t"
      "wgmma.mma_async.sync.aligned.m64n16k16.f32.f16.f16 {%0, %1, %2, %3, %4, %5, %6, %7}, %8, %9, p, 1, 1, %10, %11;\n\t}"
      : "+f"(d[0]), "+f"(d[1]), "+f"(d[2]), "+f"(d[3]), "+f"(d[4]), "+f"(d[5]), "+f"(d[6]), "+f"(d[7])
      : "l"(adesc), "l"(bdesc), "n"(TA), "n"(TB)
      : "memory");
}
template <int TA, int TB>
__device__ __forceinline__ void wgmma_n64(float* d, uint64_t adesc, uint64_t bdesc) {
  asm volatile(
      "{\n\t.reg .pred p;\n\tsetp.ne.b32 p, 1, 0;\n\t"
      "wgmma.mma_async.sync.aligned.m64n64k16.f32.f16.f16 {%0, %1, %2, %3, %4, %5, %6, %7, %8, %9, %10, %11, %12, %13, %14, %15, %16, %17, %18, %19, %20, %21, %22, %23, %24, %25, %26, %27, %28, %29, %30, %31}, %32, %33, p, 1, 1, %34, %35;\n\t}"
      : "+f"(d[0]), "+f"(d[1]), "+f"(d[2]), "+f"(d[3]), "+f"(d[4]), "+f"(d[5]), "+f"(d[6]), "+f"(d[7]), "+f"(d[8]), "+f"(d[9]), "+f"(d[10]), "+f"(d[11]), "+f"(d[12]), "+f"(d[13]), "+f"(d[14]), "+f"(d[15]), "+f"(d[16]), "+f"(d[17]), "+f"(d[18]), "+f"(d[19]), "+f"(d[20]), "+f"(d[21]), "+f"(d[22]), "+f"(d[23]), "+f"(d[24]), "+f"(d[25]), "+f"(d[26]), "+f"(d[27]), "+f"(d[28]), "+f"(d[29]), "+f"(d[30]), "+f"(d[31])
      : "l"(adesc), "l"(bdesc), "n"(TA), "n"(TB)
      : "memory");
}
template <int TA, int TB>
__device__ __forceinline__ void wgmma_n128(float* d, uint64_t adesc, uint64_t bdesc) {
  asm volatile(
      "{\n\t.reg .pred p;\n\tsetp.ne.b32 p, 1, 0;\n\t"
      "wgmma.mma_async.sync.aligned.m64n128k16.f32.f16.f16 {%0, %1, %2, %3, %4, %5, %6, %7, %8, %9, %10, %11, %12, %13, %14, %15, %16, %17, %18, %19, %20, %21, %22, %23, %24, %25, %26, %27, %28, %29, %30, %31, %32, %33, %34, %35, %36, %37, %38, %39, %40, %41, %42, %43, %44, %45, %46, %47, %48, %49, %50, %51, %52, %53, %54, %55, %56, %57, %58, %59, %60, %61, %62, %63}, %64, %65, p, 1, 1, %66, %67;\n\t}"
      : "+f"(d[0]), "+f"(d[1]), "+f"(d[2]), "+f"(d[3]), "+f"(d[4]), "+f"(d[5]), "+f"(d[6]), "+f"(d[7]), "+f"(d[8]), "+f"(d[9]), "+f"(d[10]), "+f"(d[11]), "+f"(d[12]), "+f"(d[13]), "+f"(d[14]), "+f"(d[15]), "+f"(d[16]), "+f"(d[17]), "+f"(d[18]), "+f"(d[19]), "+f"(d[20]), "+f"(d[21]), "+f"(d[22]), "+f"(d[23]), "+f"(d[24]), "+f"(d[25]), "+f"(d[26]), "+f"(d[27]), "+f"(d[28]), "+f"(d[29]), "+f"(d[30]), "+f"(d[31]), "+f"(d[32]), "+f"(d[33]), "+f"(d[34]), "+f"(d[35]), "+f"(d[36]), "+f"(d[37]), "+f"(d[38]), "+f"(d[39]), "+f"(d[40]), "+f"(d[41]), "+f"(d[42]), "+f"(d[43]), "+f"(d[44]), "+f"(d[45]), "+f"(d[46]), "+f"(d[47]), "+f"(d[48]), "+f"(d[49]), "+f"(d[50]), "+f"(d[51]), "+f"(d[52]), "+f"(d[53]), "+f"(d[54]), "+f"(d[55]), "+f"(d[56]), "+f"(d[57]), "+f"(d[58]), "+f"(d[59]), "+f"(d[60]), "+f"(d[61]), "+f"(d[62]), "+f"(d[63])
      : "l"(adesc), "l"(bdesc), "n"(TA), "n"(TB)
      : "memory");
}
template <int TA, int TB>
__device__ __forceinline__ void wgmma_n192(float* d, uint64_t adesc, uint64_t bdesc) {
  asm volatile(
      "{\n\t.reg .pred p;\n\tsetp.ne.b32 p, 1, 0;\n\t"
      "wgmma.mma_async.sync.aligned.m64n192k16.f32.f16.f16 {%0, %1, %2, %3, %4, %5, %6, %7, %8, %9, %10, %11, %12, %13, %14, %15, %16, %17, %18, %19, %20, %21, %22, %23, %24, %25, %26, %27, %28, %29, %30, %31, %32, %33, %34, %35, %36, %37, %38, %39, %40, %41, %42, %43, %44, %45, %46, %47, %48, %49, %50, %51, %52, %53, %54, %55, %56, %57, %58, %59, %60, %61, %62, %63, %64, %65, %66, %67, %68, %69, %70, %71, %72, %73, %74, %75, %76, %77, %78, %79, %80, %81, %82, %83, %84, %85, %86, %87, %88, %89, %90, %91, %92, %93, %94, %95}, %96, %97, p, 1, 1, %98, %99;\n\t}"
      : "+f"(d[0]), "+f"(d[1]), "+f"(d[2]), "+f"(d[3]), "+f"(d[4]), "+f"(d[5]), "+f"(d[6]), "+f"(d[7]), "+f"(d[8]), "+f"(d[9]), "+f"(d[10]), "+f"(d[11]), "+f"(d[12]), "+f"(d[13]), "+f"(d[14]), "+f"(d[15]), "+f"(d[16]), "+f"(d[17]), "+f"(d[18]), "+f"(d[19]), "+f"(d[20]), "+f"(d[21]), "+f"(d[22]), "+f"(d[23]), "+f"(d[24]), "+f"(d[25]), "+f"(d[26]), "+f"(d[27]), "+f"(d[28]), "+f"(d[29]), "+f"(d[30]), "+f"(d[31]), "+f"(d[32]), "+f"(d[33]), "+f"(d[34]), "+f"(d[35]), "+f"(d[36]), "+f"(d[37]), "+f"(d[38]), "+f"(d[39]), "+f"(d[40]), "+f"(d[41]), "+f"(d[42]), "+f"(d[43]), "+f"(d[44]), "+f"(d[45]), "+f"(d[46]), "+f"(d[47]), "+f"(d[48]), "+f"(d[49]), "+f"(d[50]), "+f"(d[51]), "+f"(d[52]), "+f"(d[53]), "+f"(d[54]), "+f"(d[55]), "+f"(d[56]), "+f"(d[57]), "+f"(d[58]), "+f"(d[59]), "+f"(d[60]), "+f"(d[61]), "+f"(d[62]), "+f"(d[63]), "+f"(d[64]), "+f"(d[65]), "+f"(d[66]), "+f"(d[67]), "+f"(d[68]), "+f"(d[69]), "+f"(d[70]), "+f"(d[71]), "+f"(d[72]), "+f"(d[73]), "+f"(d[74]), "+f"(d[75]), "+f"(d[76]), "+f"(d[77]), "+f"(d[78]), "+f"(d[79]), "+f"(d[80]), "+f"(d[81]), "+f"(d[82]), "+f"(d[83]), "+f"(d[84]), "+f"(d[85]), "+f"(d[86]), "+f"(d[87]), "+f"(d[88]), "+f"(d[89]), "+f"(d[90]), "+f"(d[91]), "+f"(d[92]), "+f"(d[93]), "+f"(d[94]), "+f"(d[95])
      : "l"(adesc), "l"(bdesc), "n"(TA), "n"(TB)
      : "memory");
}
template <int TA, int TB>
__device__ __forceinline__ void wgmma_n256(float* d, uint64_t adesc, uint64_t bdesc) {
  asm volatile(
      "{\n\t.reg .pred p;\n\tsetp.ne.b32 p, 1, 0;\n\t"
      "wgmma.mma_async.sync.aligned.m64n256k16.f32.f16.f16 {%0, %1, %2, %3, %4, %5, %6, %7, %8, %9, %10, %11, %12, %13, %14, %15, %16, %17, %18, %19, %20, %21, %22, %23, %24, %25, %26, %27, %28, %29, %30, %31, %32, %33, %34, %35, %36, %37, %38, %39, %40, %41, %42, %43, %44, %45, %46, %47, %48, %49, %50, %51, %52, %53, %54, %55, %56, %57, %58, %59, %60, %61, %62, %63, %64, %65, %66, %67, %68, %69, %70, %71, %72, %73, %74, %75, %76, %77, %78, %79, %80, %81, %82, %83, %84, %85, %86, %87, %88, %89, %90, %91, %92, %93, %94, %95, %96, %97, %98, %99, %100, %101, %102, %103, %104, %105, %106, %107, %108, %109, %110, %111, %112, %113, %114, %115, %116, %117, %118, %119, %120, %121, %122, %123, %124, %125, %126, %127}, %128, %129, p, 1, 1, %130, %131;\n\t}"
      : "+f"(d[0]), "+f"(d[1]), "+f"(d[2]), "+f"(d[3]), "+f"(d[4]), "+f"(d[5]), "+f"(d[6]), "+f"(d[7]), "+f"(d[8]), "+f"(d[9]), "+f"(d[10]), "+f"(d[11]), "+f"(d[12]), "+f"(d[13]), "+f"(d[14]), "+f"(d[15]), "+f"(d[16]), "+f"(d[17]), "+f"(d[18]), "+f"(d[19]), "+f"(d[20]), "+f"(d[21]), "+f"(d[22]), "+f"(d[23]), "+f"(d[24]), "+f"(d[25]), "+f"(d[26]), "+f"(d[27]), "+f"(d[28]), "+f"(d[29]), "+f"(d[30]), "+f"(d[31]), "+f"(d[32]), "+f"(d[33]), "+f"(d[34]), "+f"(d[35]), "+f"(d[36]), "+f"(d[37]), "+f"(d[38]), "+f"(d[39]), "+f"(d[40]), "+f"(d[41]), "+f"(d[42]), "+f"(d[43]), "+f"(d[44]), "+f"(d[45]), "+f"(d[46]), "+f"(d[47]), "+f"(d[48]), "+f"(d[49]), "+f"(d[50]), "+f"(d[51]), "+f"(d[52]), "+f"(d[53]), "+f"(d[54]), "+f"(d[55]), "+f"(d[56]), "+f"(d[57]), "+f"(d[58]), "+f"(d[59]), "+f"(d[60]), "+f"(d[61]), "+f"(d[62]), "+f"(d[63]), "+f"(d[64]), "+f"(d[65]), "+f"(d[66]), "+f"(d[67]), "+f"(d[68]), "+f"(d[69]), "+f"(d[70]), "+f"(d[71]), "+f"(d[72]), "+f"(d[73]), "+f"(d[74]), "+f"(d[75]), "+f"(d[76]), "+f"(d[77]), "+f"(d[78]), "+f"(d[79]), "+f"(d[80]), "+f"(d[81]), "+f"(d[82]), "+f"(d[83]), "+f"(d[84]), "+f"(d[85]), "+f"(d[86]), "+f"(d[87]), "+f"(d[88]), "+f"(d[89]), "+f"(d[90]), "+f"(d[91]), "+f"(d[92]), "+f"(d[93]), "+f"(d[94]), "+f"(d[95]), "+f"(d[96]), "+f"(d[97]), "+f"(d[98]), "+f"(d[99]), "+f"(d[100]), "+f"(d[101]), "+f"(d[102]), "+f"(d[103]), "+f"(d[104]), "+f"(d[105]), "+f"(d[106]), "+f"(d[107]), "+f"(d[108]), "+f"(d[109]), "+f"(d[110]), "+f"(d[111]), "+f"(d[112]), "+f"(d[113]), "+f"(d[114]), "+f"(d[115]), "+f"(d[116]), "+f"(d[117]), "+f"(d[118]), "+f"(d[119]), "+f"(d[120]), "+f"(d[121]), "+f"(d[122]), "+f"(d[123]), "+f"(d[124]), "+f"(d[125]), "+f"(d[126]), "+f"(d[127])
      : "l"(adesc), "l"(bdesc), "n"(TA), "n"(TB)
      : "memory");
}
template <int TA, int TB>
__device__ __forceinline__ void wgmma_n32(float* d, uint64_t adesc, uint64_t bdesc) {
  asm volatile(
      "{\n\t.reg .pred p;\n\tsetp.ne.b32 p, 1, 0;\n\t"
      "wgmma.mma_async.sync.aligned.m64n32k16.f32.f16.f16 {%0, %1, %2, %3, %4, %5, %6, %7, %8, %9, %10, %11, %12, %13, %14, %15}, %16, %17, p, 1, 1, %18, %19;\n\t}"
      : "+f"(d[0]), "+f"(d[1]), "+f"(d[2]), "+f"(d[3]), "+f"(d[4]), "+f"(d[5]), "+f"(d[6]), "+f"(d[7]), "+f"(d[8]), "+f"(d[9]), "+f"(d[10]), "+f"(d[11]), "+f"(d[12]), "+f"(d[13]), "+f"(d[14]), "+f"(d[15])
      : "l"(adesc), "l"(bdesc), "n"(TA), "n"(TB)
      : "memory");
}
template <int TA, int TB>
__device__ __forceinline__ void wgmma_n48(float* d, uint64_t adesc, uint64_t bdesc) {
  asm volatile(
      "{\n\t.reg .pred p;\n\tsetp.ne.b32 p, 1, 0;\n\t"
      "wgmma.mma_async.sync.aligned.m64n48k16.f32.f16.f16 {%0, %1, %2, %3, %4, %5, %6, %7, %8, %9, %10, %11, %12, %13, %14, %15, %16, %17, %18, %19, %20, %21, %22, %23}, %24, %25, p, 1, 1, %26, %27;\n\t}"
      : "+f"(d[0]), "+f"(d[1]), "+f"(d[2]), "+f"(d[3]), "+f"(d[4]), "+f"(d[5]), "+f"(d[6]), "+f"(d[7]), "+f"(d[8]), "+f"(d[9]), "+f"(d[10]), "+f"(d[11]), "+f"(d[12]), "+f"(d[13]), "+f"(d[14]), "+f"(d[15]), "+f"(d[16]), "+f"(d[17]), "+f"(d[18]), "+f"(d[19]), "+f"(d[20]), "+f"(d[21]), "+f"(d[22]), "+f"(d[23])
      : "l"(adesc), "l"(bdesc), "n"(TA), "n"(TB)
      : "memory");
}
template <int TA, int TB>
__device__ __forceinline__ void wgmma_n80(float* d, uint64_t adesc, uint64_t bdesc) {
  asm volatile(
      "{\n\t.reg .pred p;\n\tsetp.ne.b32 p, 1, 0;\n\t"
      "wgmma.mma_async.sync.aligned.m64n80k16.f32.f16.f16 {%0, %1, %2, %3, %4, %5, %6, %7, %8, %9, %10, %11, %12, %13, %14, %15, %16, %17, %18, %19, %20, %21, %22, %23, %24, %25, %26, %27, %28, %29, %30, %31, %32, %33, %34, %35, %36, %37, %38, %39}, %40, %41, p, 1, 1, %42, %43;\n\t}"
      : "+f"(d[0]), "+f"(d[1]), "+f"(d[2]), "+f"(d[3]), "+f"(d[4]), "+f"(d[5]), "+f"(d[6]), "+f"(d[7]), "+f"(d[8]), "+f"(d[9]), "+f"(d[10]), "+f"(d[11]), "+f"(d[12]), "+f"(d[13]), "+f"(d[14]), "+f"(d[15]), "+f"(d[16]), "+f"(d[17]), "+f"(d[18]), "+f"(d[19]), "+f"(d[20]), "+f"(d[21]), "+f"(d[22]), "+f"(d[23]), "+f"(d[24]), "+f"(d[25]), "+f"(d[26]), "+f"(d[27]), "+f"(d[28]), "+f"(d[29]), "+f"(d[30]), "+f"(d[31]), "+f"(d[32]), "+f"(d[33]), "+f"(d[34]), "+f"(d[35]), "+f"(d[36]), "+f"(d[37]), "+f"(d[38]), "+f"(d[39])
      : "l"(adesc), "l"(bdesc), "n"(TA), "n"(TB)
      : "memory");
}
template <int TA, int TB>
__device__ __forceinline__ void wgmma_n96(float* d, uint64_t adesc, uint64_t bdesc) {
  asm volatile(
      "{\n\t.reg .pred p;\n\tsetp.ne.b32 p, 1, 0;\n\t"
      "wgmma.mma_async.sync.aligned.m64n96k16.f32.f16.f16 {%0, %1, %2, %3, %4, %5, %6, %7, %8, %9, %10, %11, %12, %13, %14, %15, %16, %17, %18, %19, %20, %21, %22, %23, %24, %25, %26, %27, %28, %29, %30, %31, %32, %33, %34, %35, %36, %37, %38, %39, %40, %41, %42, %43, %44, %45, %46, %47}, %48, %49, p, 1, 1, %50, %51;\n\t}"
      : "+f"(d[0]), "+f"(d[1]), "+f"(d[2]), "+f"(d[3]), "+f"(d[4]), "+f"(d[5]), "+f"(d[6]), "+f"(d[7]), "+f"(d[8]), "+f"(d[9]), "+f"(d[10]), "+f"(d[11]), "+f"(d[12]), "+f"(d[13]), "+f"(d[14]), "+f"(d[15]), "+f"(d[16]), "+f"(d[17]), "+f"(d[18]), "+f"(d[19]), "+f"(d[20]), "+f"(d[21]), "+f"(d[22]), "+f"(d[23]), "+f"(d[24]), "+f"(d[25]), "+f"(d[26]), "+f"(d[27]), "+f"(d[28]), "+f"(d[29]), "+f"(d[30]), "+f"(d[31]), "+f"(d[32]), "+f"(d[33]), "+f"(d[34]), "+f"(d[35]), "+f"(d[36]), "+f"(d[37]), "+f"(d[38]), "+f"(d[39]), "+f"(d[40]), "+f"(d[41]), "+f"(d[42]), "+f"(d[43]), "+f"(d[44]), "+f"(d[45]), "+f"(d[46]), "+f"(d[47])
      : "l"(adesc), "l"(bdesc), "n"(TA), "n"(TB)
      : "memory");
}
template <int TA, int TB>
__device__ __forceinline__ void wgmma_n112(float* d, uint64_t adesc, uint64_t bdesc) {
  asm volatile(
      "{\n\t.reg .pred p;\n\tsetp.ne.b32 p, 1, 0;\n\t"
      "wgmma.mma_async.sync.aligned.m64n112k16.f32.f16.f16 {%0, %1, %2, %3, %4, %5, %6, %7, %8, %9, %10, %11, %12, %13, %14, %15, %16, %17, %18, %19, %20, %21, %22, %23, %24, %25, %26, %27, %28, %29, %30, %31, %32, %33, %34, %35, %36, %37, %38, %39, %40, %41, %42, %43, %44, %45, %46, %47, %48, %49, %50, %51, %52, %53, %54, %55}, %56, %57, p, 1, 1, %58, %59;\n\t}"
      : "+f"(d[0]), "+f"(d[1]), "+f"(d[2]), "+f"(d[3]), "+f"(d[4]), "+f"(d[5]), "+f"(d[6]), "+f"(d[7]), "+f"(d[8]), "+f"(d[9]), "+f"(d[10]), "+f"(d[11]), "+f"(d[12]), "+f"(d[13]), "+f"(d[14]), "+f"(d[15]), "+f"(d[16]), "+f"(d[17]), "+f"(d[18]), "+f"(d[19]), "+f"(d[20]), "+f"(d[21]), "+f"(d[22]), "+f"(d[23]), "+f"(d[24]), "+f"(d[25]), "+f"(d[26]), "+f"(d[27]), "+f"(d[28]), "+f"(d[29]), "+f"(d[30]), "+f"(d[31]), "+f"(d[32]), "+f"(d[33]), "+f"(d[34]), "+f"(d[35]), "+f"(d[36]), "+f"(d[37]), "+f"(d[38]), "+f"(d[39]), "+f"(d[40]), "+f"(d[41]), "+f"(d[42]), "+f"(d[43]), "+f"(d[44]), "+f"(d[45]), "+f"(d[46]), "+f"(d[47]), "+f"(d[48]), "+f"(d[49]), "+f"(d[50]), "+f"(d[51]), "+f"(d[52]), "+f"(d[53]), "+f"(d[54]), "+f"(d[55])
      : "l"(adesc), "l"(bdesc), "n"(TA), "n"(TB)
      : "memory");
}
template <int N, int TA, int TB>
__device__ __forceinline__ void wgmma(float* d, uint64_t adesc, uint64_t bdesc) {
  static_assert((N % 16 == 0 && N <= 128) || N == 192 || N == 256, "wgmma N");
  if constexpr (N == 16) wgmma_n16<TA, TB>(d, adesc, bdesc);
  else if constexpr (N == 32) wgmma_n32<TA, TB>(d, adesc, bdesc);
  else if constexpr (N == 48) wgmma_n48<TA, TB>(d, adesc, bdesc);
  else if constexpr (N == 64) wgmma_n64<TA, TB>(d, adesc, bdesc);
  else if constexpr (N == 80) wgmma_n80<TA, TB>(d, adesc, bdesc);
  else if constexpr (N == 96) wgmma_n96<TA, TB>(d, adesc, bdesc);
  else if constexpr (N == 112) wgmma_n112<TA, TB>(d, adesc, bdesc);
  else if constexpr (N == 128) wgmma_n128<TA, TB>(d, adesc, bdesc);
  else if constexpr (N == 192) wgmma_n192<TA, TB>(d, adesc, bdesc);
  else wgmma_n256<TA, TB>(d, adesc, bdesc);
}

__device__ __forceinline__ void producer_regs() { asm volatile("setmaxnreg.dec.sync.aligned.u32 40;"); }
__device__ __forceinline__ void consumer_regs() { asm volatile("setmaxnreg.inc.sync.aligned.u32 232;"); }
__device__ __forceinline__ void named_bar_sync(int id, int threads) { asm volatile("bar.sync %0, %1;" ::"r"(id), "r"(threads) : "memory"); }
__device__ __forceinline__ void named_bar_arrive(int id, int threads) { asm volatile("bar.arrive %0, %1;" ::"r"(id), "r"(threads) : "memory"); }

}
}
```

### action-detection_b200/csrc/umma_epi32.cuh

```cuda
#pragma once
#include "umma_conv.cuh"
#include "umma_dev.cuh"

namespace ssnb {
namespace umma {

struct U8 { uint32_t v[8]; };
__device__ __forceinline__ U8 ldg256(const void* p) {
  const uint4 a = reinterpret_cast<const uint4*>(p)[0], b = reinterpret_cast<const uint4*>(p)[1];
  return U8{{a.x, a.y, a.z, a.w, b.x, b.y, b.z, b.w}};
}
__device__ __forceinline__ U8 ldg256_nc(const void* p) {
  const uint4 a = __ldg(reinterpret_cast<const uint4*>(p)), b = __ldg(reinterpret_cast<const uint4*>(p) + 1);
  return U8{{a.x, a.y, a.z, a.w, b.x, b.y, b.z, b.w}};
}
__device__ __forceinline__ void stg256(void* p, const U8& a) {
  reinterpret_cast<uint4*>(p)[0] = make_uint4(a.v[0], a.v[1], a.v[2], a.v[3]);
  reinterpret_cast<uint4*>(p)[1] = make_uint4(a.v[4], a.v[5], a.v[6], a.v[7]);
}

__device__ __forceinline__ void store_chunk32(const UmmaConvParams& p, float alpha, const uint32_t* r, const float* bias, float* dst, __half* hdst,
                                              const float* ymask, long long lo_off) {
  float v[16];
#pragma unroll
  for (int j = 0; j < 16; ++j) v[j] = __uint_as_float(r[j]) * alpha;
  if (p.bias) {
#pragma unroll
    for (int j = 0; j < 4; ++j) {
      const float4 b = __ldg(reinterpret_cast<const float4*>(bias) + j);
      v[4 * j] += b.x; v[4 * j + 1] += b.y; v[4 * j + 2] += b.z; v[4 * j + 3] += b.w;
    }
  }
  if (p.accumulate) {
    const U8 o0 = ldg256(dst), o1 = ldg256(dst + 8);
#pragma unroll
    for (int j = 0; j < 8; ++j) { v[j] += __uint_as_float(o0.v[j]); v[8 + j] += __uint_as_float(o1.v[j]); }
  }
  if (p.relu) {
#pragma unroll
    for (int j = 0; j < 16; ++j) v[j] = fmaxf(v[j], 0.f);
  }
  if (ymask) {
    const U8 y0 = ldg256_nc(ymask), y1 = ldg256_nc(ymask + 8);
#pragma unroll
    for (int j = 0; j < 8; ++j) {
      if (!(__uint_as_float(y0.v[j]) > 0.f)) v[j] = 0.f;
      if (!(__uint_as_float(y1.v[j]) > 0.f)) v[8 + j] = 0.f;
    }
  }
  U8 q0, q1;
#pragma unroll
  for (int j = 0; j < 8; ++j) { q0.v[j] = __float_as_uint(v[j]); q1.v[j] = __float_as_uint(v[8 + j]); }
  stg256(dst, q0);
  stg256(dst + 8, q1);
  if (hdst) {
    if (p.flag || p.plane_scale != 1.0f) {
      float m = 0.f;
#pragma unroll
      for (int j = 0; j < 16; ++j) { v[j] *= p.plane_scale; m = fmaxf(m, fabsf(v[j])); if (v[j] != v[j]) m = INFINITY; }
      if (p.flag && !(m <= 65504.f)) *p.flag = 1;
    }
    U8 qh, ql;
#pragma unroll
    for (int j = 0; j < 8; ++j) {
      const __half2 h = __floats2half2_rn(v[2 * j], v[2 * j + 1]);
      const float2 hf = __half22float2(h);
      const __half2 l = __floats2half2_rn(v[2 * j] - hf.x, v[2 * j + 1] - hf.y);
      qh.v[j] = *reinterpret_cast<const uint32_t*>(&h);
      ql.v[j] = *reinterpret_cast<const uint32_t*>(&l);
    }
    stg256(hdst, qh);
    stg256(reinterpret_cast<char*>(hdst) + lo_off, ql);
  }
}

}
}
```

Baseline: 587.7.

## Move conv epilogue to register-side math with swizzled smem staging and TMA stores

The epilogue now applies alpha, bias, accumulate, relu and mask directly on the wgmma accumulator fragments, then writes the results into swizzled shared-memory tiles. One thread issues 4D TMA bulk stores for the f32 output and the optional hi/lo f16 planes, replacing per-thread row-chunk global stores. Each output and mask-plane target gets its own tensor map, and mask binding can now fail and report an error. This should cut epilogue global-store overhead and let stores overlap with the next tile. In exchange it removes output-stride sampling support and uses more epilogue shared memory.

```diff
diff --git a/action-detection_b200/csrc/engine.cu b/action-detection_b200/csrc/engine.cu
--- a/action-detection_b200/csrc/engine.cu
+++ b/action-detection_b200/csrc/engine.cu
@@ -803,8 +803,12 @@
       else if (c.kind == OP_CONV && c.fuse_role == 0 && c.umma_dgrad.enabled) dg = &c.umma_dgrad;
       if (dg) {
         c.dgrad_masks = true;
-        if (h->exact_tc()) umma_conv_set_mask_tc(*dg, h->view((int)v, false), h->planes((int)v, true), gs, h->tc_flag);
-        else umma_conv_set_mask(*dg, h->view((int)v, false));
+        if (h->exact_tc()) {
+          if (int rc = umma_conv_set_mask_tc(h->umma_ctx, *dg, h->view((int)v, false), h->planes((int)v, true), gs, h->tc_flag))
+            return h->fail(rc, "mask bind(" + h->vals[v].name + "): " + ssnb::thread_error());
+        } else {
+          umma_conv_set_mask(*dg, h->view((int)v, false));
+        }
       } else if (c.kind == OP_GPOOL && h->fast()) {
         c.dgrad_masks = true;
       }
diff --git a/action-detection_b200/csrc/umma_conv.cu b/action-detection_b200/csrc/umma_conv.cu
--- a/action-detection_b200/csrc/umma_conv.cu
+++ b/action-detection_b200/csrc/umma_conv.cu
@@ -5,7 +5,6 @@
 
 #include "umma_conv.cuh"
 #include "umma_dev.cuh"
-#include "umma_epi32.cuh"
 
 namespace ssnb {
 
@@ -19,8 +18,9 @@
 constexpr int N_STEP = 16;
 constexpr int MAX_BLOCK_N = 128;
 constexpr int EPI_COLS = 16;
-constexpr int EPI_PITCH = EPI_COLS + 4;
-constexpr int EPI_BYTES = BLOCK_M * EPI_PITCH * 4;
+constexpr int EPI_F32_BYTES = BLOCK_M * EPI_COLS * 4;
+constexpr int EPI_F16_BYTES = BLOCK_M * EPI_COLS * 2;
+constexpr int EPI_BYTES = EPI_F32_BYTES + 2 * EPI_F16_BYTES;
 constexpr int BAR_BYTES = 256;
 constexpr int SMEM_BYTES = PIPE_BYTES + 2 * EPI_BYTES + BAR_BYTES + 1024 ;
 constexpr int ORDER_BAR = 1;
@@ -39,80 +39,10 @@
   return t;
 }
 
-__device__ __forceinline__ void epilogue_chunk(const UmmaConvParams& p, const uint32_t* r, int col, uint4* dst, const uint4& o0,
-                                               const uint4& o1, const uint4& y0, const uint4& y1) {
-  float v[16];
-#pragma unroll
-  for (int j = 0; j < 16; ++j) v[j] = __uint_as_float(r[j]);
-  if (p.bias) {
-#pragma unroll
-    for (int j = 0; j < 16; ++j) v[j] += __ldg(p.bias + col + j);
-  }
-  if (p.accumulate) {
-    const __half2* h0 = reinterpret_cast<const __half2*>(&o0);
-    const __half2* h1 = reinterpret_cast<const __half2*>(&o1);
-#pragma unroll
-    for (int j = 0; j < 4; ++j) {
-      float2 a = __half22float2(h0[j]), b = __half22float2(h1[j]);
-      v[2 * j] += a.x; v[2 * j + 1] += a.y; v[8 + 2 * j] += b.x; v[8 + 2 * j + 1] += b.y;
-    }
-  }
-  if (p.relu) {
-#pragma unroll
-    for (int j = 0; j < 16; ++j) v[j] = fmaxf(v[j], 0.f);
-  }
-  if (p.mask_y) {
-    const __half2* a0 = reinterpret_cast<const __half2*>(&y0);
-    const __half2* a1 = reinterpret_cast<const __half2*>(&y1);
-#pragma unroll
-    for (int j = 0; j < 4; ++j) {
-      const float2 ya = __half22float2(a0[j]), yb = __half22float2(a1[j]);
-      if (!(ya.x > 0.f)) v[2 * j] = 0.f;
-      if (!(ya.y > 0.f)) v[2 * j + 1] = 0.f;
-      if (!(yb.x > 0.f)) v[8 + 2 * j] = 0.f;
-      if (!(yb.y > 0.f)) v[8 + 2 * j + 1] = 0.f;
-    }
-  }
-  uint4 q0, q1;
-  __half2* g0 = reinterpret_cast<__half2*>(&q0);
-  __half2* g1 = reinterpret_cast<__half2*>(&q1);
-#pragma unroll
-  for (int j = 0; j < 4; ++j) { g0[j] = __floats2half2_rn(v[2 * j], v[2 * j + 1]); g1[j] = __floats2half2_rn(v[8 + 2 * j], v[8 + 2 * j + 1]); }
-  dst[0] = q0; dst[1] = q1;
-}
-
-__device__ __forceinline__ void epilogue_row_chunk(const UmmaConvParams& p, const TileCoord& t, int row, int col, const float* st) {
-  const int rw = row % p.bw, rh = (row / p.bw) % p.bh, rf = row / (p.bw * p.bh);
-  const int w = t.w0 + rw, h = t.h0 + rh, f = t.f0 + rf;
-  const int os = p.out_stride;
-  const bool valid = (rf < p.bf) && (w < p.W) && (h < p.H) && (f < p.F) && (w % os == 0) && (h % os == 0);
-  if (!valid || col >= p.Cout) return;
-  const long long opix = (long long)(f * p.OH + h / os) * p.OW + w / os;
-  uint32_t r[16];
-#pragma unroll
-  for (int j = 0; j < 4; ++j) {
-    const float4 q = reinterpret_cast<const float4*>(st)[j];
-    r[4 * j] = __float_as_uint(q.x); r[4 * j + 1] = __float_as_uint(q.y); r[4 * j + 2] = __float_as_uint(q.z); r[4 * j + 3] = __float_as_uint(q.w);
-  }
-  const bool d1 = col < p.n_split;
-  if (p.out_f32) {
-    const float alpha = p.alpha * (p.alpha_dev ? __ldg(p.alpha_dev) : 1.0f);
-    float* o32 = d1 ? p.out32 + opix * p.out_pitch + p.out_coff + col : p.out32_2 + opix * p.out2_pitch + p.out2_coff - p.n_split + col;
-    __half* hi = d1 ? p.out_hi : p.out_hi2;
-    if (hi) hi += d1 ? opix * p.out_pitch + p.out_coff + col : opix * p.out2_pitch + p.out2_coff - p.n_split + col;
-    const float* m32 = p.mask32 ? p.mask32 + opix * p.mask32_pitch + p.mask32_coff + col : nullptr;
-    store_chunk32(p, alpha, r, p.bias + col, o32, hi, m32, d1 ? p.out_lo_off : p.out_lo_off2);
-    return;
-  }
-  uint4* dst = reinterpret_cast<uint4*>(d1 ? p.out + opix * p.out_pitch + p.out_coff + col : p.out2 + opix * p.out2_pitch + p.out2_coff - p.n_split + col);
-  uint4 o0 = {}, o1 = {}, y0 = {}, y1 = {};
-  if (p.accumulate) { o0 = dst[0]; o1 = dst[1]; }
-  if (p.mask_y) {
-    const uint4* my = reinterpret_cast<const uint4*>(p.mask_y + opix * p.mask_pitch + p.mask_coff + col);
-    y0 = __ldg(my); y1 = __ldg(my + 1);
-  }
-  epilogue_chunk(p, r, col, dst, o0, o1, y0, y1);
-}
+__device__ __forceinline__ uint32_t sw64_off(int r, int c) { return r * 64 + ((((c >> 2) ^ (r >> 1)) & 3) << 4) + (c & 3) * 4; }
+__device__ __forceinline__ uint32_t sw32_off(int r, int c) { return r * 32 + ((((c >> 3) ^ (r >> 2)) & 1) << 4) + (c & 7) * 2; }
+
+__device__ __forceinline__ uint32_t h2_bits(__half2 h) { return *reinterpret_cast<const uint32_t*>(&h); }
 
 template <int BN, int NK>
 __device__ __forceinline__ void mma_k(float* d0, float* d1, uint32_t sa, uint32_t sb) {
@@ -144,6 +74,9 @@
 umma_conv_kernel(const __grid_constant__ CUtensorMap tmap_a, const __grid_constant__ CUtensorMap tmap_a2,
                  const __grid_constant__ CUtensorMap tmap_b, const __grid_constant__ CUtensorMap tmap_a_lo,
                  const __grid_constant__ CUtensorMap tmap_a2_lo, const __grid_constant__ CUtensorMap tmap_b_lo,
+                 const __grid_constant__ CUtensorMap tmap_o, const __grid_constant__ CUtensorMap tmap_o_hi,
+                 const __grid_constant__ CUtensorMap tmap_o_lo, const __grid_constant__ CUtensorMap tmap_o2,
+                 const __grid_constant__ CUtensorMap tmap_o2_hi, const __grid_constant__ CUtensorMap tmap_o2_lo,
                  const __grid_constant__ UmmaConvParams p) {
   extern __shared__ uint8_t smem_raw[];
   uint8_t* smem = reinterpret_cast<uint8_t*>((reinterpret_cast<uintptr_t>(smem_raw) + 1023) & ~(uintptr_t)1023);
@@ -163,6 +96,7 @@
     asm volatile("prefetch.tensormap [%0];" ::"l"(reinterpret_cast<uint64_t>(&tmap_a)) : "memory");
     asm volatile("prefetch.tensormap [%0];" ::"l"(reinterpret_cast<uint64_t>(&tmap_a2)) : "memory");
     asm volatile("prefetch.tensormap [%0];" ::"l"(reinterpret_cast<uint64_t>(&tmap_b)) : "memory");
+    asm volatile("prefetch.tensormap [%0];" ::"l"(reinterpret_cast<uint64_t>(&tmap_o)) : "memory");
     for (int i = 0; i < STAGES; ++i) { mbar_init(&full_bar[i], 1); mbar_init(&empty_bar[i], 1); }
     asm volatile("fence.mbarrier_init.release.cluster;" ::: "memory");
   }
@@ -200,7 +134,8 @@
     consumer_regs();
     const int cw = wg - 1, row = threadIdx.x & 127;
     const int warp = row / 32, lane = row & 31;
-    float* epi = reinterpret_cast<float*>(smem + PIPE_BYTES + cw * EPI_BYTES);
+    uint8_t* epi = smem + PIPE_BYTES + cw * EPI_BYTES;
+    const float alpha = p.out_f32 ? p.alpha * (p.alpha_dev ? __ldg(p.alpha_dev) : 1.0f) : 1.0f;
     const int my_tiles = (total_tiles - (int)blockIdx.x + (int)gridDim.x - 1) / (int)gridDim.x;
     uint32_t stage = 0, phase = 0;
     if (cw) ring_advance(stage, phase, ksteps, STAGES);
@@ -238,26 +173,186 @@
       wgmma_wait<0>();
       if (row == 0) mbar_arrive(&empty_bar[prev]);
       ring_advance(stage, phase, ksteps, STAGES);
-#pragma unroll
-      for (int sl = 0; sl < (BN + EPI_COLS - 1) / EPI_COLS; ++sl) {
+      bool rv[2][2];
+      int rpix[2][2];
+#pragma unroll
+      for (int b = 0; b < 2; ++b)
+#pragma unroll
+        for (int h = 0; h < 2; ++h) {
+          const int r = b * 64 + warp * 16 + (lane >> 2) + 8 * h;
+          const int rw = r % p.bw, rh = (r / p.bw) % p.bh, rf = r / (p.bw * p.bh);
+          const int w = t.w0 + rw, y = t.h0 + rh, f = t.f0 + rf;
+          rv[b][h] = rf < p.bf && w < p.W && y < p.H && f < p.F;
+          rpix[b][h] = (f * p.H + y) * p.W + w;
+        }
+      const int q2 = 2 * (lane & 3);
+#pragma unroll
+      for (int sl = 0; sl < BN / EPI_COLS; ++sl) {
+        const int col = t.n0 + sl * EPI_COLS;
+        if (col >= p.Cout) break;
+        const bool d1 = col < p.n_split;
+        const int cd = d1 ? col : col - p.n_split;
+        const int opitch = d1 ? p.out_pitch : p.out2_pitch, ocoff = d1 ? p.out_coff : p.out2_coff;
+        float v[2][2][4];
+#pragma unroll
+        for (int b = 0; b < 2; ++b)
+#pragma unroll
+          for (int h = 0; h < 2; ++h)
+#pragma unroll
+            for (int k = 0; k < 2; ++k) {
+              const int i = sl * (EPI_COLS / 2) + 4 * k + 2 * h;
+              v[b][h][2 * k] = acc[b][i]; v[b][h][2 * k + 1] = acc[b][i + 1];
+            }
+        const bool planes = p.out_f32 && (d1 ? p.planes : p.planes2);
+        if (p.out_f32) {
+#pragma unroll
+          for (int b = 0; b < 2; ++b)
+#pragma unroll
+            for (int h = 0; h < 2; ++h)
+#pragma unroll
+              for (int j = 0; j < 4; ++j) v[b][h][j] = __fmul_rn(v[b][h][j], alpha);
+          if (p.bias) {
+#pragma unroll
+            for (int k = 0; k < 2; ++k) {
+              const float2 bb = __ldg(reinterpret_cast<const float2*>(p.bias + col + 8 * k + q2));
+#pragma unroll
+              for (int b = 0; b < 2; ++b)
+#pragma unroll
+                for (int h = 0; h < 2; ++h) { v[b][h][2 * k] = __fadd_rn(v[b][h][2 * k], bb.x); v[b][h][2 * k + 1] = __fadd_rn(v[b][h][2 * k + 1], bb.y); }
+            }
+          }
+          if (p.accumulate) {
+            const float* o32 = (d1 ? p.out32 : p.out32_2) + ocoff + cd + q2;
+#pragma unroll
+            for (int b = 0; b < 2; ++b)
+#pragma unroll
+              for (int h = 0; h < 2; ++h)
+                if (rv[b][h])
+#pragma unroll
+                  for (int k = 0; k < 2; ++k) {
+                    const float2 o = *reinterpret_cast<const float2*>(o32 + (long long)rpix[b][h] * opitch + 8 * k);
+                    v[b][h][2 * k] = __fadd_rn(v[b][h][2 * k], o.x); v[b][h][2 * k + 1] = __fadd_rn(v[b][h][2 * k + 1], o.y);
+                  }
+          }
+          if (p.relu) {
+#pragma unroll
+            for (int b = 0; b < 2; ++b)
+#pragma unroll
+              for (int h = 0; h < 2; ++h)
+#pragma unroll
+                for (int j = 0; j < 4; ++j) v[b][h][j] = fmaxf(v[b][h][j], 0.f);
+          }
+          if (p.mask32) {
+            const float* m32 = p.mask32 + p.mask32_coff + col + q2;
+#pragma unroll
+            for (int b = 0; b < 2; ++b)
+#pragma unroll
+              for (int h = 0; h < 2; ++h)
+#pragma unroll
+                for (int k = 0; k < 2; ++k) {
+                  const float2 y = rv[b][h] ? __ldg(reinterpret_cast<const float2*>(m32 + (long long)rpix[b][h] * p.mask32_pitch + 8 * k)) : make_float2(0.f, 0.f);
+                  if (!(y.x > 0.f)) v[b][h][2 * k] = 0.f;
+                  if (!(y.y > 0.f)) v[b][h][2 * k + 1] = 0.f;
+                }
+          }
+        } else {
+          if (p.bias) {
+#pragma unroll
+            for (int k = 0; k < 2; ++k) {
+              const float2 bb = __ldg(reinterpret_cast<const float2*>(p.bias + col + 8 * k + q2));
+#pragma unroll
+              for (int b = 0; b < 2; ++b)
+#pragma unroll
+                for (int h = 0; h < 2; ++h) { v[b][h][2 * k] += bb.x; v[b][h][2 * k + 1] += bb.y; }
+            }
+          }
+          if (p.accumulate) {
+            const __half* o16 = (d1 ? p.out : p.out2) + ocoff + cd + q2;
+#pragma unroll
+            for (int b = 0; b < 2; ++b)
+#pragma unroll
+              for (int h = 0; h < 2; ++h)
+                if (rv[b][h])
+#pragma unroll
+                  for (int k = 0; k < 2; ++k) {
+                    const float2 o = __half22float2(*reinterpret_cast<const __half2*>(o16 + (long long)rpix[b][h] * opitch + 8 * k));
+                    v[b][h][2 * k] += o.x; v[b][h][2 * k + 1] += o.y;
+                  }
+          }
+          if (p.relu) {
+#pragma unroll
+            for (int b = 0; b < 2; ++b)
+#pragma unroll
+              for (int h = 0; h < 2; ++h)
+#pragma unroll
+                for (int j = 0; j < 4; ++j) v[b][h][j] = fmaxf(v[b][h][j], 0.f);
+          }
+          if (p.mask_y) {
+            const __half* my = p.mask_y + p.mask_coff + col + q2;
+#pragma unroll
+            for (int b = 0; b < 2; ++b)
+#pragma unroll
+              for (int h = 0; h < 2; ++h)
+#pragma unroll
+                for (int k = 0; k < 2; ++k) {
+                  const float2 y = rv[b][h] ? __half22float2(__ldg(reinterpret_cast<const __half2*>(my + (long long)rpix[b][h] * p.mask_pitch + 8 * k)))
+                                            : make_float2(0.f, 0.f);
+                  if (!(y.x > 0.f)) v[b][h][2 * k] = 0.f;
+                  if (!(y.y > 0.f)) v[b][h][2 * k + 1] = 0.f;
+                }
+          }
+        }
+        if (row == 0) bulk_wait_read0();
         named_bar_sync(EPI_BAR + cw, 128);
+        const bool scaled = p.flag || p.plane_scale != 1.0f;
+        float m = 0.f;
 #pragma unroll
         for (int b = 0; b < 2; ++b)
 #pragma unroll
-          for (int i = 0; i < EPI_COLS / 2; i += 2) {
-            const int ai = sl * (EPI_COLS / 2) + i;
-            if (ai < BN / 2) {
-              const int r = b * 64 + warp * 16 + (lane >> 2) + 8 * ((i >> 1) & 1);
-              const int c = 8 * (i >> 2) + 2 * (lane & 3);
-              *reinterpret_cast<float2*>(epi + r * EPI_PITCH + c) = make_float2(acc[b][ai], acc[b][ai + 1]);
+          for (int h = 0; h < 2; ++h) {
+            const int r = b * 64 + warp * 16 + (lane >> 2) + 8 * h;
+            if (p.out_f32) {
+              const bool s = (lane >> 3) & 1;
+              const float2 x0 = make_float2(v[b][h][0], v[b][h][1]), x1 = make_float2(v[b][h][2], v[b][h][3]);
+              *reinterpret_cast<float2*>(epi + sw64_off(r, q2 + (s ? 8 : 0))) = s ? x1 : x0;
+              *reinterpret_cast<float2*>(epi + sw64_off(r, q2 + (s ? 0 : 8))) = s ? x0 : x1;
+              if (planes)
+#pragma unroll
+                for (int k = 0; k < 2; ++k) {
+                  float x0 = v[b][h][2 * k], x1 = v[b][h][2 * k + 1];
+                  if (scaled) {
+                    x0 = __fmul_rn(x0, p.plane_scale); x1 = __fmul_rn(x1, p.plane_scale);
+                    if (rv[b][h]) {
+                      m = fmaxf(m, fabsf(x0)); if (x0 != x0) m = INFINITY;
+                      m = fmaxf(m, fabsf(x1)); if (x1 != x1) m = INFINITY;
+                    }
+                  }
+                  const __half2 hh = __floats2half2_rn(x0, x1);
+                  const float2 hf = __half22float2(hh);
+                  *reinterpret_cast<uint32_t*>(epi + EPI_F32_BYTES + sw32_off(r, 8 * k + q2)) = h2_bits(hh);
+                  *reinterpret_cast<uint32_t*>(epi + EPI_F32_BYTES + EPI_F16_BYTES + sw32_off(r, 8 * k + q2)) =
+                      h2_bits(__floats2half2_rn(__fsub_rn(x0, hf.x), __fsub_rn(x1, hf.y)));
+                }
+            } else {
+#pragma unroll
+              for (int k = 0; k < 2; ++k)
+                *reinterpret_cast<uint32_t*>(epi + sw32_off(r, 8 * k + q2)) = h2_bits(__floats2half2_rn(v[b][h][2 * k], v[b][h][2 * k + 1]));
             }
           }
+        if (planes && p.flag && !(m <= 65504.f)) *p.flag = 1;
+        fence_proxy_async_smem();
         named_bar_sync(EPI_BAR + cw, 128);
-#pragma unroll
-        for (int c = 0; c < EPI_COLS; c += 16)
-          if (sl * EPI_COLS + c < BN) epilogue_row_chunk(p, t, row, t.n0 + sl * EPI_COLS + c, epi + row * EPI_PITCH + c);
+        if (row == 0) {
+          tma_store_4d(d1 ? &tmap_o : &tmap_o2, epi, cd, t.w0, t.h0, t.f0);
+          if (planes) {
+            tma_store_4d(d1 ? &tmap_o_hi : &tmap_o2_hi, epi + EPI_F32_BYTES, cd, t.w0, t.h0, t.f0);
+            tma_store_4d(d1 ? &tmap_o_lo : &tmap_o2_lo, epi + EPI_F32_BYTES + EPI_F16_BYTES, cd, t.w0, t.h0, t.f0);
+          }
+          bulk_commit();
+        }
       }
     }
+    if (row == 0) bulk_wait0();
   }
 }
 
@@ -283,10 +378,11 @@
 }
 
 int encode(UmmaContext& ctx, CUtensorMap* m, int rank, void* addr, const cuuint64_t* dims, const cuuint64_t* strides,
-           const cuuint32_t* box, int spatial_stride = 1) {
+           const cuuint32_t* box, int spatial_stride = 1, CUtensorMapDataType dtype = CU_TENSOR_MAP_DATA_TYPE_FLOAT16,
+           CUtensorMapSwizzle swizzle = CU_TENSOR_MAP_SWIZZLE_128B) {
   cuuint32_t es[5] = {1, (cuuint32_t)spatial_stride, (cuuint32_t)spatial_stride, 1, 1};
-  CUresult r = reinterpret_cast<EncodeTiledFn>(ctx.encode_tiled)(m, CU_TENSOR_MAP_DATA_TYPE_FLOAT16, (cuuint32_t)rank, addr, dims, strides,
-                                                                box, es, CU_TENSOR_MAP_INTERLEAVE_NONE, CU_TENSOR_MAP_SWIZZLE_128B,
+  CUresult r = reinterpret_cast<EncodeTiledFn>(ctx.encode_tiled)(m, dtype, (cuuint32_t)rank, addr, dims, strides,
+                                                                box, es, CU_TENSOR_MAP_INTERLEAVE_NONE, swizzle,
                                                                 CU_TENSOR_MAP_L2_PROMOTION_L2_256B, CU_TENSOR_MAP_FLOAT_OOB_FILL_NONE);
   if (r != CUDA_SUCCESS) {
     char buf[128];
@@ -305,13 +401,43 @@
   else { bw = 1; bh = 1; bf = 128; }
 }
 
-int bind_common(UmmaContext& ctx, UmmaConvPlan& plan, View a, View o, int F, int K, int N, int ntaps, int out_stride, const __half* w,
+int encode_out(UmmaContext& ctx, CUtensorMap* m, const UmmaConvParams& p, const void* base, int pitch, int n, bool f32) {
+  const cuuint64_t es = f32 ? 4 : 2;
+  cuuint64_t dims[4] = {(cuuint64_t)n, (cuuint64_t)p.W, (cuuint64_t)p.H, (cuuint64_t)p.F};
+  cuuint64_t str[3] = {(cuuint64_t)pitch * es, (cuuint64_t)p.W * pitch * es, (cuuint64_t)p.H * p.W * pitch * es};
+  cuuint32_t box[4] = {(cuuint32_t)EPI_COLS, (cuuint32_t)p.bw, (cuuint32_t)p.bh, (cuuint32_t)p.bf};
+  return encode(ctx, m, 4, const_cast<void*>(base), dims, str, box, 1, f32 ? CU_TENSOR_MAP_DATA_TYPE_FLOAT32 : CU_TENSOR_MAP_DATA_TYPE_FLOAT16,
+                f32 ? CU_TENSOR_MAP_SWIZZLE_64B : CU_TENSOR_MAP_SWIZZLE_32B);
+}
+
+int encode_planes(UmmaContext& ctx, CUtensorMap* mhi, CUtensorMap* mlo, const UmmaConvParams& p, const __half* hi, long long lo_off, int pitch, int n) {
+  if (int rc = encode_out(ctx, mhi, p, hi, pitch, n, false)) return rc;
+  return encode_out(ctx, mlo, p, reinterpret_cast<const char*>(hi) + lo_off, pitch, n, false);
+}
+
+int bind_out(UmmaContext& ctx, UmmaConvPlan& plan, View o, float* out32, int n, bool second) {
+  UmmaConvParams& p = plan.p;
+  CUtensorMap* m = second ? &plan.tmap_o2 : &plan.tmap_o;
+  CUtensorMap* mhi = second ? &plan.tmap_o2_hi : &plan.tmap_o_hi;
+  CUtensorMap* mlo = second ? &plan.tmap_o2_lo : &plan.tmap_o_lo;
+  const bool f32 = p.out_f32 != 0;
+  if (int rc = encode_out(ctx, m, p, f32 ? (const void*)(out32 + o.coff) : (const void*)(reinterpret_cast<__half*>(o.base) + o.coff), o.pitch, n, f32))
+    return rc;
+  *mhi = *m; *mlo = *m;
+  const int planes = f32 && o.base;
+  if (planes)
+    if (int rc = encode_planes(ctx, mhi, mlo, p, reinterpret_cast<__half*>(o.base) + o.coff, o.lo_off, o.pitch, n)) return rc;
+  (second ? p.planes2 : p.planes) = planes;
+  return 0;
+}
+
+int bind_common(UmmaContext& ctx, UmmaConvPlan& plan, View a, View o, int F, int K, int N, int ntaps, const __half* w,
                 int a_stride = 1, const UmmaTcOpts* tc = nullptr) {
   plan.enabled = false;
   if (int rc = resolve_encode(ctx)) return rc;
   if (a_stride == 2) {
     View ao = a; ao.H = o.H; ao.W = o.W;
-    if (int rc = bind_common(ctx, plan, ao, o, F, K, N, ntaps, 1, w, 1, tc)) return rc;
+    if (int rc = bind_common(ctx, plan, ao, o, F, K, N, ntaps, w, 1, tc)) return rc;
     plan.enabled = false;
     UmmaConvParams& q = plan.p;
     q.a_stride = 2;
@@ -326,7 +452,7 @@
     plan.enabled = true;
     return 0;
   }
-  if ((a.H + out_stride - 1) / out_stride != o.H || (a.W + out_stride - 1) / out_stride != o.W) { set_thread_error("umma conv: geometry mismatch"); return 1; }
+  if (a.H != o.H || a.W != o.W) { set_thread_error("umma conv: geometry mismatch"); return 1; }
   if (K % 8 || N % 16 || a.pitch % 8 || a.coff % 8 || o.pitch % 8 || o.coff % 8 || ntaps > UMMA_MAX_TAPS) {
     set_thread_error("umma conv: unsupported channel alignment"); return 1; }
   UmmaConvParams& p = plan.p;
@@ -340,7 +466,7 @@
   p.K = K;
   p.ntaps = ntaps;
   p.out = reinterpret_cast<__half*>(o.base); p.out_pitch = o.pitch; p.out_coff = o.coff; p.Cout = N;
-  p.out_stride = out_stride; p.OH = o.H; p.OW = o.W; p.a_stride = 1; p.mask_y = nullptr; p.mask_pitch = 0; p.mask_coff = 0;
+  p.a_stride = 1; p.mask_y = nullptr; p.mask_pitch = 0; p.mask_coff = 0;
   p.kchunks_a1 = (K + BLOCK_K - 1) / BLOCK_K; p.K1 = K; p.n_split = 1 << 30; p.out2 = p.out; p.out2_pitch = o.pitch; p.out2_coff = o.coff;
   {
     cuuint64_t dims[4] = {(cuuint64_t)K, (cuuint64_t)a.W, (cuuint64_t)a.H, (cuuint64_t)F};
@@ -367,9 +493,11 @@
   p.stages = PIPE_BYTES / p.stage_bytes; if (p.stages > MAX_STAGES) p.stages = MAX_STAGES;
   p.alpha = tc ? tc->alpha : 1.0f; p.alpha_dev = tc ? tc->alpha_dev : nullptr;
   p.mask32 = nullptr; p.mask32_pitch = 0; p.mask32_coff = 0; p.plane_scale = 1.0f; p.flag = nullptr;
-  p.out32 = tc ? tc->out32 : nullptr; p.out_hi = tc ? reinterpret_cast<__half*>(o.base) : nullptr; p.out_lo_off = tc ? o.lo_off : 0;
-  p.out32_2 = p.out32; p.out_hi2 = p.out_hi; p.out_lo_off2 = p.out_lo_off;
+  p.out32 = tc ? tc->out32 : nullptr;
   if (tc && (!tc->out32 || !a.lo_off || !tc->w_lo_off)) { set_thread_error("umma conv: split-operand bind needs operand planes and an fp32 output"); return 1; }
+  if (int rc = bind_out(ctx, plan, o, p.out32, N, false)) return rc;
+  p.out32_2 = p.out32; p.planes2 = p.planes;
+  plan.tmap_o2 = plan.tmap_o; plan.tmap_o2_hi = plan.tmap_o_hi; plan.tmap_o2_lo = plan.tmap_o_lo;
   plan.enabled = true;
   return 0;
 }
@@ -377,7 +505,7 @@
 void mark_tc_ok(UmmaConvPlan& plan, int W, bool two_sources) {
   UmmaConvParams& p = plan.p;
   p.tc_ok = 0;
-  if (!plan.enabled || p.a_stride != 1 || p.out_stride != 1) return;
+  if (!plan.enabled || p.a_stride != 1) return;
   if (!(p.ntaps == 1 || p.ntaps == 4 || p.ntaps == 9)) return;
   if (p.kchunks_a1 != p.kchunks && (p.ntaps != 1 || !two_sources)) return;
   if (p.out_pitch % 16 || p.out_coff % 16 || p.out2_pitch % 16 || p.out2_coff % 16 || p.n_split % 16 || (p.bias && p.n_tiles * p.block_n > 1024)) return;
@@ -398,7 +526,7 @@
 
 int umma_conv_bind_taps(UmmaContext& ctx, UmmaConvPlan& plan, View in, View out, int F, int cin, int cout, int ntaps,
                         const int* dy, const int* dx, const __half* w_tap_n_k, const float* bias, int relu, const UmmaTcOpts* tc) {
-  if (int rc = bind_common(ctx, plan, in, out, F, cin, cout, ntaps, 1, w_tap_n_k, 1, tc)) return rc;
+  if (int rc = bind_common(ctx, plan, in, out, F, cin, cout, ntaps, w_tap_n_k, 1, tc)) return rc;
   for (int t = 0; t < ntaps; ++t) { plan.p.tap_dy[t] = dy[t]; plan.p.tap_dx[t] = dx[t]; }
   plan.p.bias = bias; plan.p.relu = relu; plan.p.accumulate = 0;
   mark_tc_ok(plan, in.W, false);
@@ -407,10 +535,8 @@
 
 int umma_conv_bind_fwd(UmmaContext& ctx, UmmaConvPlan& plan, View in, View out, int F, int cin, int cout, int k, int pad,
                        int stride, const __half* w_tap_n_k, const float* bias, const UmmaTcOpts* tc) {
-  const char* st = getenv("SSNB_TMA_STRIDED");
-  const bool strided = stride == 2 && !(st && st[0] == '0');
-  if (int rc = strided ? bind_common(ctx, plan, in, out, F, cin, cout, k * k, 1, w_tap_n_k, 2, tc)
-                       : bind_common(ctx, plan, in, out, F, cin, cout, k * k, stride, w_tap_n_k, 1, tc)) return rc;
+  if (stride != 1 && stride != 2) { set_thread_error("umma conv: stride must be 1 or 2"); return 1; }
+  if (int rc = bind_common(ctx, plan, in, out, F, cin, cout, k * k, w_tap_n_k, stride, tc)) return rc;
   for (int r = 0; r < k; ++r)
     for (int s = 0; s < k; ++s) { plan.p.tap_dy[r * k + s] = r - pad; plan.p.tap_dx[r * k + s] = s - pad; }
   plan.p.bias = bias; plan.p.relu = 1; plan.p.accumulate = 0;
@@ -420,7 +546,7 @@
 
 int umma_conv_bind_dgrad(UmmaContext& ctx, UmmaConvPlan& plan, View dz, View dx, int F, int cin, int cout, int k, int pad,
                          const __half* w_tap_k_n, int accumulate, const UmmaTcOpts* tc) {
-  if (int rc = bind_common(ctx, plan, dz, dx, F, cout, cin, k * k, 1, w_tap_k_n, 1, tc)) return rc;
+  if (int rc = bind_common(ctx, plan, dz, dx, F, cout, cin, k * k, w_tap_k_n, 1, tc)) return rc;
   for (int r = 0; r < k; ++r)
     for (int s = 0; s < k; ++s) { plan.p.tap_dy[r * k + s] = pad - r; plan.p.tap_dx[r * k + s] = pad - s; }
   plan.p.bias = nullptr; plan.p.relu = 0; plan.p.accumulate = accumulate;
@@ -432,14 +558,14 @@
                              const __half* w_n_k, const float* bias, const UmmaTcOpts* tc) {
   View o = out1; o.C = n1 + n2;
   if (out1.H != out2.H || out1.W != out2.W || n1 % 16 || n2 % 16 || out2.pitch % 8 || out2.coff % 8) { set_thread_error("fused fwd: bad views"); return 1; }
-  if (int rc = bind_common(ctx, plan, in, o, F, cin, n1 + n2, 1, 1, w_n_k, 1, tc)) return rc;
+  if (tc && !tc->out32_2) { set_thread_error("fused fwd: the split-operand bind needs both fp32 destinations"); return 1; }
+  if (int rc = bind_common(ctx, plan, in, o, F, cin, n1 + n2, 1, w_n_k, 1, tc)) return rc;
   plan.p.tap_dy[0] = 0; plan.p.tap_dx[0] = 0;
   plan.p.bias = bias; plan.p.relu = 1; plan.p.accumulate = 0;
   plan.p.n_split = n1; plan.p.out2 = reinterpret_cast<__half*>(out2.base); plan.p.out2_pitch = out2.pitch; plan.p.out2_coff = out2.coff;
-  if (tc) {
-    if (!tc->out32_2) { set_thread_error("fused fwd: the split-operand bind needs both fp32 destinations"); return 1; }
-    plan.p.out32_2 = tc->out32_2; plan.p.out_hi2 = reinterpret_cast<__half*>(out2.base); plan.p.out_lo_off2 = out2.lo_off;
-  }
+  if (tc) plan.p.out32_2 = tc->out32_2;
+  if (int rc = bind_out(ctx, plan, out1, plan.p.out32, n1, false)) { plan.enabled = false; return rc; }
+  if (int rc = bind_out(ctx, plan, out2, plan.p.out32_2, n2, true)) { plan.enabled = false; return rc; }
   mark_tc_ok(plan, in.W, false);
   return 0;
 }
@@ -448,7 +574,7 @@
                                const __half* w_n_k, int accumulate, const UmmaTcOpts* tc) {
   const int k1p = (k1 + BLOCK_K - 1) / BLOCK_K * BLOCK_K;
   View a = k1 ? dz1 : dz2;
-  if (int rc = bind_common(ctx, plan, a, dx, F, k1 ? k1 : k2, cin, 1, 1, w_n_k, 1, tc)) return rc;
+  if (int rc = bind_common(ctx, plan, a, dx, F, k1 ? k1 : k2, cin, 1, w_n_k, 1, tc)) return rc;
   UmmaConvParams& p = plan.p;
   p.tap_dy[0] = 0; p.tap_dx[0] = 0; p.bias = nullptr; p.relu = 0; p.accumulate = accumulate;
   if (k1) {
@@ -481,15 +607,17 @@
   plan.mask_y = reinterpret_cast<const __half*>(y.base); plan.mask_pitch = y.pitch; plan.mask_coff = y.coff;
 }
 
-void umma_conv_set_mask_tc(UmmaConvPlan& plan, View y32, View dplanes, float plane_scale, int* flag) {
+int umma_conv_set_mask_tc(UmmaContext& ctx, UmmaConvPlan& plan, View y32, View dplanes, float plane_scale, int* flag) {
+  if (int rc = encode_planes(ctx, &plan.tmap_mask_hi, &plan.tmap_mask_lo, plan.p, reinterpret_cast<__half*>(dplanes.base) + dplanes.coff, dplanes.lo_off,
+                             dplanes.pitch, plan.p.Cout)) return rc;
   plan.mask32 = reinterpret_cast<const float*>(y32.base); plan.mask32_pitch = y32.pitch; plan.mask32_coff = y32.coff;
-  plan.mask_planes = reinterpret_cast<__half*>(dplanes.base); plan.mask_planes_lo = dplanes.lo_off;
-  plan.mask_plane_scale = plane_scale; plan.mask_flag = flag;
+  plan.mask_planes = true; plan.mask_plane_scale = plane_scale; plan.mask_flag = flag;
+  return 0;
 }
 
 namespace {
 template <int BN>
-int launch_bn(const UmmaConvPlan& plan, const UmmaConvParams& p, int grid, cudaStream_t s) {
+int launch_bn(const UmmaConvPlan& plan, const UmmaConvParams& p, const CUtensorMap& o_hi, const CUtensorMap& o_lo, int grid, cudaStream_t s) {
   static bool attr_set[64] = {};
   auto kern = umma_conv_kernel<BN>;
   int dev = 0;
@@ -499,7 +627,8 @@
       set_thread_error("umma conv: cannot raise dynamic shared memory limit"); cudaGetLastError(); return 2; }
     if (dev >= 0 && dev < 64) attr_set[dev] = true;
   }
-  kern<<<grid, NUM_THREADS, SMEM_BYTES, s>>>(plan.tmap_a, plan.tmap_a2, plan.tmap_b, plan.tmap_a_lo, plan.tmap_a2_lo, plan.tmap_b_lo, p);
+  kern<<<grid, NUM_THREADS, SMEM_BYTES, s>>>(plan.tmap_a, plan.tmap_a2, plan.tmap_b, plan.tmap_a_lo, plan.tmap_a2_lo, plan.tmap_b_lo, plan.tmap_o, o_hi, o_lo,
+                                             plan.tmap_o2, plan.tmap_o2_hi, plan.tmap_o2_lo, p);
   SSNB_LAUNCH_CHECK("umma_conv_kernel");
   return 0;
 }
@@ -509,23 +638,26 @@
   if (!plan.enabled) { set_thread_error("umma conv: plan not bound"); return 3; }
   UmmaConvParams p = plan.p;
   if (mask && plan.mask_y) { p.mask_y = plan.mask_y; p.mask_pitch = plan.mask_pitch; p.mask_coff = plan.mask_coff; }
-  if (mask && p.out_f32 && plan.mask32) {
+  const bool mplanes = mask && p.out_f32 && plan.mask32 && plan.mask_planes;
+  if (mplanes) {
     p.mask32 = plan.mask32; p.mask32_pitch = plan.mask32_pitch; p.mask32_coff = plan.mask32_coff;
-    p.out_hi = plan.mask_planes; p.out_lo_off = plan.mask_planes_lo; p.plane_scale = plan.mask_plane_scale; p.flag = plan.mask_flag;
-  }
-  if (p.out_f32 && (p.mask_y || p.out_stride != 1)) { set_thread_error("umma conv: the fp32 epilogue takes its mask through mask32 and has no sampling"); return 3; }
+    p.planes = 1; p.plane_scale = plan.mask_plane_scale; p.flag = plan.mask_flag;
+  }
+  if (p.out_f32 && p.mask_y) { set_thread_error("umma conv: the fp32 epilogue takes its mask through mask32"); return 3; }
+  const CUtensorMap& o_hi = mplanes ? plan.tmap_mask_hi : plan.tmap_o_hi;
+  const CUtensorMap& o_lo = mplanes ? plan.tmap_mask_lo : plan.tmap_o_lo;
   const int total = p.tiles_w * p.tiles_h * p.tiles_f * p.n_tiles;
   const int grid = total < ctx.num_sms ? total : ctx.num_sms;
   t_tag.tiles = total; t_tag.block_n = p.block_n;
   switch (p.block_n) {
-    case 16: return launch_bn<16>(plan, p, grid, s);
-    case 32: return launch_bn<32>(plan, p, grid, s);
-    case 48: return launch_bn<48>(plan, p, grid, s);
-    case 64: return launch_bn<64>(plan, p, grid, s);
-    case 80: return launch_bn<80>(plan, p, grid, s);
-    case 96: return launch_bn<96>(plan, p, grid, s);
-    case 112: return launch_bn<112>(plan, p, grid, s);
-    case 128: return launch_bn<128>(plan, p, grid, s);
+    case 16: return launch_bn<16>(plan, p, o_hi, o_lo, grid, s);
+    case 32: return launch_bn<32>(plan, p, o_hi, o_lo, grid, s);
+    case 48: return launch_bn<48>(plan, p, o_hi, o_lo, grid, s);
+    case 64: return launch_bn<64>(plan, p, o_hi, o_lo, grid, s);
+    case 80: return launch_bn<80>(plan, p, o_hi, o_lo, grid, s);
+    case 96: return launch_bn<96>(plan, p, o_hi, o_lo, grid, s);
+    case 112: return launch_bn<112>(plan, p, o_hi, o_lo, grid, s);
+    case 128: return launch_bn<128>(plan, p, o_hi, o_lo, grid, s);
   }
   set_thread_error("umma conv: unsupported tile width"); return 3;
 }
diff --git a/action-detection_b200/csrc/umma_conv.cuh b/action-detection_b200/csrc/umma_conv.cuh
--- a/action-detection_b200/csrc/umma_conv.cuh
+++ b/action-detection_b200/csrc/umma_conv.cuh
@@ -23,7 +23,6 @@
   int kchunks, ntaps, K;
   int tap_dy[UMMA_MAX_TAPS], tap_dx[UMMA_MAX_TAPS];
   __half* out; int out_pitch, out_coff, Cout;
-  int out_stride, OH, OW;
   int a_stride;
   const float* bias;
   int relu, accumulate;
@@ -35,8 +34,8 @@
   int nseg, out_f32;
   float alpha;
   const float* alpha_dev;
-  float* out32; __half* out_hi; long long out_lo_off;
-  float* out32_2; __half* out_hi2; long long out_lo_off2;
+  float* out32; int planes;
+  float* out32_2; int planes2;
   const float* mask32; int mask32_pitch, mask32_coff;
   float plane_scale; int* flag;
 };
@@ -47,8 +46,9 @@
   CUtensorMap tmap_a, tmap_a2, tmap_b;
   CUtensorMap tmap_a_lo, tmap_a2_lo, tmap_b_lo;
   long long b_lo_off = 0;
+  CUtensorMap tmap_o, tmap_o_hi, tmap_o_lo, tmap_o2, tmap_o2_hi, tmap_o2_lo;
   const float* mask32 = nullptr; int mask32_pitch = 0, mask32_coff = 0;
-  __half* mask_planes = nullptr; long long mask_planes_lo = 0; float mask_plane_scale = 1.0f; int* mask_flag = nullptr;
+  CUtensorMap tmap_mask_hi, tmap_mask_lo; bool mask_planes = false; float mask_plane_scale = 1.0f; int* mask_flag = nullptr;
   UmmaConvParams p;
 };
 
@@ -67,7 +67,7 @@
                                const __half* w_n_k, int accumulate, const UmmaTcOpts* tc = nullptr);
 int umma_conv_launch(UmmaContext& ctx, const UmmaConvPlan& plan, cudaStream_t s, bool mask = false);
 void umma_conv_set_mask(UmmaConvPlan& plan, View y);
-void umma_conv_set_mask_tc(UmmaConvPlan& plan, View y32, View dplanes, float plane_scale, int* flag);
+int umma_conv_set_mask_tc(UmmaContext& ctx, UmmaConvPlan& plan, View y32, View dplanes, float plane_scale, int* flag);
 
 int umma_resolve_encode(UmmaContext& ctx);
 int umma_encode_f16(UmmaContext& ctx, CUtensorMap* m, int rank, void* addr, const cuuint64_t* dims,
diff --git a/action-detection_b200/csrc/umma_dev.cuh b/action-detection_b200/csrc/umma_dev.cuh
--- a/action-detection_b200/csrc/umma_dev.cuh
+++ b/action-detection_b200/csrc/umma_dev.cuh
@@ -56,6 +56,16 @@
       "l"(reinterpret_cast<uint64_t>(map)), "r"(smem_u32(bar)), "r"(c0), "r"(c1), "r"(c2)
       : "memory");
 }
+
+__device__ __forceinline__ void tma_store_4d(const CUtensorMap* map, const void* src, int c0, int c1, int c2, int c3) {
+  asm volatile("cp.async.bulk.tensor.4d.global.shared::cta.bulk_group [%0, {%2, %3, %4, %5}], [%1];" ::"l"(reinterpret_cast<uint64_t>(map)),
+               "r"(smem_u32(src)), "r"(c0), "r"(c1), "r"(c2), "r"(c3)
+               : "memory");
+}
+__device__ __forceinline__ void bulk_commit() { asm volatile("cp.async.bulk.commit_group;" ::: "memory"); }
+__device__ __forceinline__ void bulk_wait_read0() { asm volatile("cp.async.bulk.wait_group.read 0;" ::: "memory"); }
+__device__ __forceinline__ void bulk_wait0() { asm volatile("cp.async.bulk.wait_group 0;" ::: "memory"); }
+__device__ __forceinline__ void fence_proxy_async_smem() { asm volatile("fence.proxy.async.shared::cta;" ::: "memory"); }
 
 __device__ __forceinline__ uint64_t make_desc_sw128(uint32_t saddr, uint32_t lbo_bytes = 16) {
   uint64_t d = 0;
diff --git a/action-detection_b200/csrc/umma_epi32.cuh b/action-detection_b200/csrc/umma_epi32.cuh
--- a/action-detection_b200/csrc/umma_epi32.cuh
+++ /dev/null
@@ -1,78 +0,0 @@
-#pragma once
-#include "umma_conv.cuh"
-#include "umma_dev.cuh"
-
-namespace ssnb {
-namespace umma {
-
-struct U8 { uint32_t v[8]; };
-__device__ __forceinline__ U8 ldg256(const void* p) {
-  const uint4 a = reinterpret_cast<const uint4*>(p)[0], b = reinterpret_cast<const uint4*>(p)[1];
-  return U8{{a.x, a.y, a.z, a.w, b.x, b.y, b.z, b.w}};
-}
-__device__ __forceinline__ U8 ldg256_nc(const void* p) {
-  const uint4 a = __ldg(reinterpret_cast<const uint4*>(p)), b = __ldg(reinterpret_cast<const uint4*>(p) + 1);
-  return U8{{a.x, a.y, a.z, a.w, b.x, b.y, b.z, b.w}};
-}
-__device__ __forceinline__ void stg256(void* p, const U8& a) {
-  reinterpret_cast<uint4*>(p)[0] = make_uint4(a.v[0], a.v[1], a.v[2], a.v[3]);
-  reinterpret_cast<uint4*>(p)[1] = make_uint4(a.v[4], a.v[5], a.v[6], a.v[7]);
-}
-
-__device__ __forceinline__ void store_chunk32(const UmmaConvParams& p, float alpha, const uint32_t* r, const float* bias, float* dst, __half* hdst,
-                                              const float* ymask, long long lo_off) {
-  float v[16];
-#pragma unroll
-  for (int j = 0; j < 16; ++j) v[j] = __uint_as_float(r[j]) * alpha;
-  if (p.bias) {
-#pragma unroll
-    for (int j = 0; j < 4; ++j) {
-      const float4 b = __ldg(reinterpret_cast<const float4*>(bias) + j);
-      v[4 * j] += b.x; v[4 * j + 1] += b.y; v[4 * j + 2] += b.z; v[4 * j + 3] += b.w;
-    }
-  }
-  if (p.accumulate) {
-    const U8 o0 = ldg256(dst), o1 = ldg256(dst + 8);
-#pragma unroll
-    for (int j = 0; j < 8; ++j) { v[j] += __uint_as_float(o0.v[j]); v[8 + j] += __uint_as_float(o1.v[j]); }
-  }
-  if (p.relu) {
-#pragma unroll
-    for (int j = 0; j < 16; ++j) v[j] = fmaxf(v[j], 0.f);
-  }
-  if (ymask) {
-    const U8 y0 = ldg256_nc(ymask), y1 = ldg256_nc(ymask + 8);
-#pragma unroll
-    for (int j = 0; j < 8; ++j) {
-      if (!(__uint_as_float(y0.v[j]) > 0.f)) v[j] = 0.f;
-      if (!(__uint_as_float(y1.v[j]) > 0.f)) v[8 + j] = 0.f;
-    }
-  }
-  U8 q0, q1;
-#pragma unroll
-  for (int j = 0; j < 8; ++j) { q0.v[j] = __float_as_uint(v[j]); q1.v[j] = __float_as_uint(v[8 + j]); }
-  stg256(dst, q0);
-  stg256(dst + 8, q1);
-  if (hdst) {
-    if (p.flag || p.plane_scale != 1.0f) {
-      float m = 0.f;
-#pragma unroll
-      for (int j = 0; j < 16; ++j) { v[j] *= p.plane_scale; m = fmaxf(m, fabsf(v[j])); if (v[j] != v[j]) m = INFINITY; }
-      if (p.flag && !(m <= 65504.f)) *p.flag = 1;
-    }
-    U8 qh, ql;
-#pragma unroll
-    for (int j = 0; j < 8; ++j) {
-      const __half2 h = __floats2half2_rn(v[2 * j], v[2 * j + 1]);
-      const float2 hf = __half22float2(h);
-      const __half2 l = __floats2half2_rn(v[2 * j] - hf.x, v[2 * j + 1] - hf.y);
-      qh.v[j] = *reinterpret_cast<const uint32_t*>(&h);
-      ql.v[j] = *reinterpret_cast<const uint32_t*>(&l);
-    }
-    stg256(hdst, qh);
-    stg256(reinterpret_cast<char*>(hdst) + lo_off, ql);
-  }
-}
-
-}
-}
```

New measurement: 668.0, median of 6. +13.7%, better.
